# scipopt/SCIP-SDP

Measured on AMD Instinct MI355X. Metric: node-SDP solves/sec, dense block n x n with m vars (IPM iters/sec in iters_per_sec), higher is better.
Workload: dtype f64

## Files before the change

### include/hipsdp_units.h

```cpp
#ifndef HIPSDP_UNITS_H
#define HIPSDP_UNITS_H

#include "hipsdp.h"

#ifdef __cplusplus
extern "C" {
#endif

HIPSDP_API int  hipsdp_dgemm_selfcheck(int device, int M, int N, int K, int layB, int batch, int splitk, int flags, double beta,
   int* used_v2, long long* ndiff);
HIPSDP_API int  hipsdp_pass_at_unit(int device, int R, long long E, const double* A, const double* coef, double sa, const double* add, int split,
   double* out, int* chunks);
HIPSDP_API int  hipsdp_dgemm_selfcheck2(int device, int M, int N, int K, int layB, int batch, int splitk, int flags, double alpha, double beta,
   int reps, int* used, long long* ndiff, double* ms_tile, double* ms_fast);
HIPSDP_API int  hipsdp_gram_plan_info(int device, int M, long long K, int nslab, int* no, int* nd, int* nitems, double* span);
HIPSDP_API int  hipsdp_gram_selfcheck(int device, int M, long long K, int reps, int* used, double* maxdiff, long long* nrepro, double* ms_tile,
   double* ms_gram);
HIPSDP_API int  hipsdp_dgemm_selfcheck3(int device, int M, int N, int K, int layB, int batch, int splitk, int flags, double alpha, double beta,
   int reps, int* used, long long* ndiff, double* maxdiff, long long* nrepro, double* ms_tile, double* ms_fast);
HIPSDP_API int  hipsdp_tri_product_unit(int device, int mode, int M, int N, int K, int layB, int batch, int flags, const double* A,
   const double* B, double* Cio, int crows, int ldc, int* used);
HIPSDP_API int  hipsdp_tri_instance_force(int mode);
HIPSDP_API int  hipsdp_schur_identity_unit(int device, int m1, int n, const double* A, double ws_gbytes, int full_storage, double* Mx,
   double* flops);
HIPSDP_API int  hipsdp_schur_dense(int device, int m1, int n, const double* A, const double* X, const double* Zinv, double* Mx,
   double ws_gbytes);
HIPSDP_API int  hipsdp_schur_w(int device, int m1, int n, const double* A, const double* X, const double* Z, double* Mx);
HIPSDP_API int  hipsdp_schur_form_unit(int device, int form, int parts, int m1, int n, const double* A, const double* P, const double* Q,
   double ws_gbytes, double* Mx, int* used);
HIPSDP_API int  hipsdp_schur_small_unit(int device, int m1, int nblk, const int* ns, const double* const* A, const double* const* X,
   const double* const* Zinv, int q, const double* Dext, const double* x, const double* z, double* Mx, double* Lm, double* diagM, int* taken);
HIPSDP_API int  hipsdp_schur_shard_time(int device, int m1, int n, int nranks, int rank, int by_columns, int reps, double ws_gbytes, double* ms);
HIPSDP_API int  hipsdp_schur_var_share_time(int device, int m1, int n, int nranks, int rank, int cw, int reps, double* ms, double* a2a_bytes);
HIPSDP_API int  hipsdp_schur_sparse_unit(int device, int n, int m, long long nnz, const int* var, const int* row, const int* col,
   const double* val, const double* X, const double* Zinv, double* Mx);
HIPSDP_API int  hipsdp_schur_sparse_unit2(int device, int n, int m, long long nnz, const int* var, const int* row, const int* col,
   const double* val, const double* X, const double* Zinv, double* Mx, int kernel, int* took);
HIPSDP_API int  hipsdp_sparse_ops_unit(int device, int n, int m, long long nnz, const int* var, const int* row, const int* col,
   const double* val, const double* V, const double* coef, const double* base, double* outA, double* outAT);
HIPSDP_API int  hipsdp_mfma_peak(int device, double ms, double* tflops, double* ghz);
HIPSDP_API int  hipsdp_potrf(int device, int n, double* A, int* fail);
HIPSDP_API int  hipsdp_potrf_ex(int device, int n, double* A, int psd, int v1, double* dinv, int* regmask, int* fail);
HIPSDP_API int  hipsdp_potrs(int device, int n, const double* A, int nrhs, double* rhs);
HIPSDP_API int  hipsdp_potrs_seq(int device, int n, const double* A, int psd, int ncalls, const int* nrhs, const int* mode, double* rhs,
   int* regmask, int* fail);
HIPSDP_API int  hipsdp_potrf_small_unit(int device, int n, int pair, const double* base, const double* dir, double alpha, int set_flag,
   int want_gram, double* L, double* dinv, double* Mout, double* Linv, double* Gram, int* flag);
HIPSDP_API long long hipsdp_potrf_dinv_len(int n);
HIPSDP_API int  hipsdp_potrf_pair_unit(int device, int n, int pair, double* A, double* dinv, int* fail);
HIPSDP_API int  hipsdp_trial_pair_unit(int device, int n, int fused, int first, double alpha, double* io);
HIPSDP_API int  hipsdp_tail_after_solve2_unit(int device, int m, int fused, const double* rhs2, const double* u1, double* u2, double* wt,
   double* e2, double* e1);
HIPSDP_API int  hipsdp_tail_unpack3_unit(int device, int n, int fused, const double* pk, double* out);
HIPSDP_API int  hipsdp_tail_dz_unit(int device, int n, int fused, const double* pk, const double* P2, const double* Rd, double dtau, double eta,
   double* dZ);
HIPSDP_API int  hipsdp_tail_dirmat_unit(int device, int n, int fused, double s1, const double* Zinv, const double* X, const double* GZ, double* H,
   double* pk);
HIPSDP_API int  hipsdp_tail_sc_len(void);
HIPSDP_API int  hipsdp_tail_dir_unit(int device, int m, int n, int fused, const double* B, const double* H, const double* rhs2, const double* rp,
   const double* b, const double* u1, const double* u2, const double* par, double* sc, double* dy, double* dyt);
HIPSDP_API int  hipsdp_tail_dots_unit(int device, int m, int n, int fused, const double* a, const double* v, double* out);
HIPSDP_API int  hipsdp_trtri(int device, int n, const double* A, double* Linv);
HIPSDP_API int  hipsdp_lambda_min(int device, int n, const double* W, int steps, double* theta, double* resid);
HIPSDP_API int  hipsdp_lambda_min_scaled(int device, int n, const double* L, const double* D, int steps, double* theta, double* resid);
HIPSDP_API int  hipsdp_solve1_fits(int m, int q, int nblk, const int* ns);
HIPSDP_API int  hipsdp_solve1_class(int m, int nblk, const int* ns);
HIPSDP_API unsigned long long hipsdp_gram_gen_next(unsigned long long* counter);
HIPSDP_API int  hipsdp_gram_key_match_unit(int m_a, int nblk_a, const int* n_a, const int* form_a, const unsigned long long* gen_a,
   const long long* ws_a, int m_b, int nblk_b, const int* n_b, const int* form_b, const unsigned long long* gen_b, const long long* ws_b);
HIPSDP_API int  hipsdp_syev_many_unit(int device, int count, const int* ns, const double* A, double* lam, double* V, int* launches);
HIPSDP_API int  hipsdp_sparsecuts_unit(int device, int count, const int* ns, const double* Z, const double* v0, const double* maxeig,
   const int* sizes, const hipsdp_sparsecut_opts* opts, int* ncuts, double* eigvals, double* vecs, int* iters, int* flags);
HIPSDP_API int  hipsdp_sparsecuts_large_unit(int device, int n, const double* Z, const double* v0, double maxeig, int size,
   const hipsdp_sparsecut_opts* opts, int* ncuts, double* eigvals, double* vecs, int* iters, int* flags);
HIPSDP_API int  hipsdp_syevx_many_below_unit(int device, int count, const int* n, const double* A, double bound, int maxk, int cap, int* cnt,
   double* lam, double* V);
HIPSDP_API int  hipsdp_tridiag_unit(int device, int n, const double* A, double* d, double* e, double* Vrefl, double* tau);
HIPSDP_API int  hipsdp_tvec_unit(int device, int n, const double* d, const double* e, double* lam, double* Z);
HIPSDP_API int  hipsdp_syevr_many_unit(int device, int count, const int* n, const double* A, int cap, double* lam, double* V);
HIPSDP_API int  hipsdp_sparse_dump_unit(hipsdp_solver* solver, int block, long long* counts, int* voff, int* vrow, int* vcol, double* vval,
   int* poff, int* prow, int* pcol, int* pvar, double* pval, int* foff, int* frow, int* fcol, double* fval, int* soff, int* srow, int* sent);
HIPSDP_API int  hipsdp_onevar_unit(int device, int n, int count, const double* Z, const double* A, const double* shift, const int* kind,
   const double* lb, const double* ub, double feastol, int maxevals, int* status, double* optval, double* lmin, double* grad, int* evals);
HIPSDP_API int  hipsdp_onevar_all_unit(int device, int count, const int* n, const double* Z, const double* A, const double* shift,
   const int* kind, const double* lb, const double* ub, double feastol, int maxevals, int mid_cap,
   int* status, double* optval, double* lmin, double* grad, int* evals);
HIPSDP_API int  hipsdp_onevar_large_unit(int device, int count, const int* n, const double* Z, const double* A, const double* shift,
   const int* kind, const double* lb, const double* ub, double feastol, int maxevals, int wg_cap, int chunk,
   int* status, double* optval, double* lmin, double* grad, int* evals, int* rounds);
HIPSDP_API int  hipsdp_objs_fanout_unit(int device, int count, int m, int q, int nblk, const int* ns, const double* B, const double* b_own,
   int have_start, const double* y, const double* x, const double* z, const double* XZ, int gap, double guard, long long* lane_len,
   long long* offs, double* lanes, int* launches);
HIPSDP_API int  hipsdp_small_dir_block_unit(int device, int n, double c, double s1, const double* X, const double* R, const double* E,
   const double* Zinv, int recorded, double* out, int* pending);
HIPSDP_API int  hipsdp_small_lp_rows_unit(int device, int q, int m1, const double* Dext, const double* v, int mode, double eta, double sigmu,
   const double* x, const double* z, const double* rd, const double* elp, int recorded, double* out1, double* out2, int* pending);
HIPSDP_API int  hipsdp_small_apply_A_unit(int device, int m1, int nblk, const int* n2, const double* A, const double* V, int q,
   const double* Dext, const double* vlp, int epi, double scal, const double* vin, int recorded, double* out, double* vout, int* pending);
HIPSDP_API int  hipsdp_small_elementwise_unit(int device, int n, const int* nn, const double* par, int use_elp, const double* in,
   const double* xs, int recorded, double* o_lp, double* o_mul, double* o_ext, double* ys, int* pending);
HIPSDP_API int  hipsdp_small_gemv_t_unit(int device, int R, long long E, long long lda, const double* A, const double* coef, double sa,
   int add_mode, const double* add, int recorded, double* out, int* pending);
HIPSDP_API int  hipsdp_reductions_unit(int device, int kind, int count, const int* len, const int* slot, const int* accumulate,
   const double* a, const double* b, const double* c, int nslots, const double* preset, int recorded, double* out, int* pending);
HIPSDP_API int  hipsdp_small_solve_unit(int device, int m, const double* M, int form, int nrhs, long long ld, double* rhs, double* u2,
   double* wt, int* pending, int* fail);
HIPSDP_API int  hipsdp_gemv_t3_unit(int device, int R, long long E, long long lda, const double* A, const double* c, int fused, double* out,
   int* took);
HIPSDP_API int  hipsdp_pass_a_unit(int device, int R, long long E, long long lda, const double* A, int nv, const double* V, int voff,
   long long wsdoubles, double* out, int* info);

#ifdef __cplusplus
}
#endif

#endif
```

### scip-sdp_amd/binding.py

```python
import ctypes as C
import os
import numpy as np

_HERE = os.path.dirname(os.path.abspath(__file__))
LIBPATH = os.environ.get("HIPSDP_LIB", os.path.join(_HERE, "lib", "libhipsdp.so"))

STATUS_NAMES = {0: "optimal", 1: "dual_infeasible", 2: "dual_unbounded", 3: "both_infeasible", 4: "iterlimit",
                5: "numeric", 6: "timelimit", 7: "objlimit", -1: "unsolved"}


class Params(C.Structure):
    _fields_ = [("gaptol", C.c_double), ("feastol", C.c_double), ("infeastol", C.c_double), ("objlimit", C.c_double),
                ("timelimit", C.c_double), ("gamma", C.c_double), ("ws_gbytes", C.c_double), ("maxiter", C.c_int),
                ("verbose", C.c_int), ("lanczos_steps", C.c_int), ("settings", C.c_int), ("pabstol", C.c_double), ("preoptgap", C.c_double)]


class Info(C.Structure):
    _fields_ = [("status", C.c_int), ("iterations", C.c_int), ("pobj", C.c_double), ("dobj", C.c_double),
                ("pinf", C.c_double), ("dinf", C.c_double), ("dabs", C.c_double), ("gap", C.c_double), ("mu", C.c_double),
                ("tau", C.c_double), ("kappa", C.c_double), ("solve_seconds", C.c_double), ("schur_seconds", C.c_double),
                ("schur_flops", C.c_double), ("schur_calls", C.c_int), ("chol_fail", C.c_int), ("warm_started", C.c_int),
                ("settings_used", C.c_int), ("schur_flops_executed", C.c_double)]


# ... 700 lines not shown

def sparsecuts_unit(ns, Zs, v0s, maxeig, sizes, feastol, maxcuts, convtol=0, maxit=0, device=0):
    ns = [int(n) for n in ns]
    cnt = len(ns)
    cns = np.asarray(ns, dtype=np.int32)
    Z = _f64(np.concatenate([np.asarray(z, dtype=np.float64).reshape(-1) for z in Zs]))
    v0 = _f64(np.concatenate([np.asarray(v, dtype=np.float64).reshape(-1) for v in v0s]))
    me = _f64(maxeig)
    sizes = np.ascontiguousarray(sizes, dtype=np.int32)
    opts = SparsecutOpts(0.0, feastol, convtol, maxcuts, maxit)
    k, it, fl = (np.zeros(cnt, dtype=np.int32) for _ in range(3))
    ev = np.zeros(cnt * maxcuts)
    ve = np.zeros(maxcuts * sum(ns))
    rc = ulib().hipsdp_sparsecuts_unit(device, cnt, _ip(cns), _dp(Z), _dp(v0), _dp(me), _ip(sizes), C.byref(opts), _ip(k), _dp(ev), _dp(ve),
                                       _ip(it), _ip(fl))
    if rc != 0:
        raise RuntimeError("hipsdp_sparsecuts_unit: %d (%s)" % (rc, ulib().hipsdp_last_error()))
    out, off = [], 0
    for j, n in enumerate(ns):
        kj = int(k[j])
        out.append((kj, ev[j * maxcuts:j * maxcuts + kj].copy(), ve[off:off + kj * n].reshape(kj, n).copy(), int(it[j]), int(fl[j])))
        off += maxcuts * n
    return out


def eigencuts_all_stats():
    calls, launches, readbacks = C.c_longlong(0), C.c_longlong(0), C.c_longlong(0)
    _chk(lib().hipsdp_eigencuts_all_stats(C.byref(calls), C.byref(launches), C.byref(readbacks)), "hipsdp_eigencuts_all_stats")
    return calls.value, launches.value, readbacks.value


def eigencuts_all_large_stats():
    calls, launches, readbacks = C.c_longlong(0), C.c_longlong(0), C.c_longlong(0)
    _chk(lib().hipsdp_eigencuts_all_large_stats(C.byref(calls), C.byref(launches), C.byref(readbacks)), "hipsdp_eigencuts_all_large_stats")
    return calls.value, launches.value, readbacks.value


def syevx_many_below_unit(mats, bound, maxk, cap, device=0):
    mats = [np.asarray(a, dtype=np.float64) for a in mats]
    ns = np.ascontiguousarray([a.shape[0] for a in mats], dtype=np.int32)
    assert all(a.shape == (n, n) for a, n in zip(mats, ns))
    cat = _f64(np.concatenate([a.reshape(-1) for a in mats]))
    cnt = np.full(len(mats), -1, dtype=np.int32)
    mk = max(1, int(maxk))
    lam = np.zeros(len(mats) * mk)
    V = np.zeros(mk * int(sum(ns)))
    rc = ulib().hipsdp_syevx_many_below_unit(device, len(mats), _ip(ns), _dp(cat), C.c_double(bound), int(maxk), int(cap), _ip(cnt), _dp(lam),
                                             _dp(V))
    if rc != 0:
        raise RuntimeError("hipsdp_syevx_many_below_unit: %d (%s)" % (rc, ulib().hipsdp_last_error()))
    out, off = [], 0
    for j, n in enumerate(ns):
        kj = int(cnt[j])
        out.append((kj, lam[j * maxk:j * maxk + kj].copy(), V[off:off + kj * n].reshape(kj, n).copy()))
        off += maxk * int(n)
    return out



def _params(kw):
    p = Params()
    lib().hipsdp_default_params(C.byref(p))
    for k, v in (kw or {}).items():
        setattr(p, k, v)
    return p


def solve_many(solvers, params=None):
    n = len(solvers)
    if isinstance(params, (list, tuple)):
        if len(params) != n:
            raise ValueError("solve_many: %d params for %d solvers" % (len(params), n))
        plist = [_params(kw) for kw in params]
    else:
        plist = [_params(params)] * n
    hs = (C.c_void_p * max(n, 1))(*[s.h for s in solvers])
    ps = (Params * max(n, 1))(*plist)
    infos = (Info * max(n, 1))()
    rcs = (C.c_int * max(n, 1))()
    rc = lib().hipsdp_solve_many(n, hs, ps, infos, rcs)
    if rc != 0:
        raise RuntimeError("hipsdp_solve_many failed: rc=%d, per solver %s (%s)" %
                           (rc, list(rcs)[:n], lib().hipsdp_last_error().decode()))
    return [infos[i] for i in range(n)]


def solve_many_stats():
    launches = C.c_longlong(0)
    problems = C.c_longlong(0)
    _chk(lib().hipsdp_solve_many_stats(C.byref(launches), C.byref(problems)), "hipsdp_solve_many_stats")
    return launches.value, problems.value


def solve_objectives_stats():
    v = [C.c_longlong(0) for _ in range(3)]
    _chk(lib().hipsdp_solve_objectives_stats(*[C.byref(x) for x in v]), "hipsdp_solve_objectives_stats")
    return tuple(x.value for x in v)


def objs_fanout_unit(B, b_own, ns, q=0, start=None, gap=2, guard=-7.25):
    B = _f64(B)
    count, m = B.shape
    b_own = _f64(b_own)
    nsa = (C.c_int * max(len(ns), 1))(*[int(n) for n in ns])
    offs = np.zeros(4 + 2 * len(ns), dtype=np.int64)
    po = offs.ctypes.data_as(C.POINTER(C.c_longlong))
    ln = C.c_longlong(0)
    launches = C.c_int(0)
    if start is not None:
        y, x, z, X, Z = start
        y, x, z = _f64(y), _f64(x if q else np.zeros(1)), _f64(z if q else np.zeros(1))
        XZ = _f64(np.concatenate([np.concatenate([_f64(X[k]).ravel(), _f64(Z[k]).ravel()]) for k in range(len(ns))]))
        ptrs = (_dp(y), _dp(x), _dp(z), _dp(XZ))
    else:
        ptrs = (None, None, None, None)
    hs = 1 if start is not None else 0
    rc = ulib().hipsdp_objs_fanout_unit(0, count, m, q, len(ns), nsa, _dp(B), _dp(b_own), hs, *ptrs, gap, C.c_double(guard), C.byref(ln),
                                        po, None, None)
    if rc != 0:
        raise RuntimeError("hipsdp_objs_fanout_unit failed: rc=%d" % rc)
    lanes = np.zeros((count + 1, ln.value))
    rc = ulib().hipsdp_objs_fanout_unit(0, count, m, q, len(ns), nsa, _dp(B), _dp(b_own), hs, *ptrs, gap, C.c_double(guard), C.byref(ln),
                                        po, _dp(lanes), C.byref(launches))
    if rc != 0:
        raise RuntimeError("hipsdp_objs_fanout_unit failed: rc=%d (%s)" % (rc, ulib().hipsdp_last_error().decode()))
    return lanes, offs.copy(), launches.value


def solve1_fits(m, q, ns):
    a = (C.c_int * max(len(ns), 1))(*[int(n) for n in ns])
    return bool(ulib().hipsdp_solve1_fits(int(m), int(q), len(ns), a))


def solve1_class(m, ns):
    a = (C.c_int * max(len(ns), 1))(*[int(n) for n in ns])
    return ulib().hipsdp_solve1_class(int(m), len(ns), a)


def dgemm(A, B, layA=0, layB=1, alpha=1.0, beta=0.0, Cin=None, lower_only=False, splitk=0, device=0):
    A = _f64(A)
    B = _f64(B)
    M, K = (A.shape if layA == 0 else A.shape[::-1])
    N = B.shape[0] if layB == 0 else B.shape[1]
    Cout = np.zeros((M, N)) if Cin is None else _f64(Cin).copy()
    _chk(lib().hipsdp_dgemm(device, layA, layB, M, N, K, C.c_double(alpha), _dp(A), C.c_longlong(A.shape[1]), _dp(B),
                            C.c_longlong(B.shape[1]), C.c_double(beta), _dp(Cout), C.c_longlong(N), int(lower_only), splitk),
         "hipsdp_dgemm")
    return Cout


def schur_dense(A, X, Zinv, ws_gbytes=0.0, device=0):
    A = _f64(A)
    m1, n = A.shape[0], A.shape[1]
    X = _f64(X)
    Zinv = _f64(Zinv)
    Mx = np.zeros((m1, m1))
    _chk(ulib().hipsdp_schur_dense(device, m1, n, _dp(A), _dp(X), _dp(Zinv), _dp(Mx), C.c_double(ws_gbytes)),
         "hipsdp_schur_dense")
    return Mx


def schur_sparse_unit(n, m, coo, X, Zinv, device=0):
    var, row, col, val = coo
    var = np.ascontiguousarray(var, dtype=np.int32); row = np.ascontiguousarray(row, dtype=np.int32)
    col = np.ascontiguousarray(col, dtype=np.int32); val = _f64(val)
    X = _f64(X); Zinv = _f64(Zinv)
    Mx = np.zeros((m + 1, m + 1))
    _chk(ulib().hipsdp_schur_sparse_unit(device, n, m, C.c_longlong(len(val)), _ip(var), _ip(row), _ip(col), _dp(val), _dp(X), _dp(Zinv), _dp(Mx)),
         "hipsdp_schur_sparse_unit")
    return Mx


def _coo_i32(coo):
    var, row, col, val = coo
    return (np.ascontiguousarray(var, dtype=np.int32), np.ascontiguousarray(row, dtype=np.int32),
            np.ascontiguousarray(col, dtype=np.int32), _f64(val))


def schur_sparse_unit2(n, m, coo, X, Zinv, kernel=-1, device=0):
    var, row, col, val = _coo_i32(coo)
    X = _f64(X); Zinv = _f64(Zinv)
    Mx = np.zeros((m + 1, m + 1))
    took = C.c_int(-7)
    _chk(ulib().hipsdp_schur_sparse_unit2(device, n, m, C.c_longlong(len(val)), _ip(var), _ip(row), _ip(col), _dp(val), _dp(X), _dp(Zinv),
                                          _dp(Mx), int(kernel), C.byref(took)), "hipsdp_schur_sparse_unit2")
    return Mx, took.value


def sparse_ops_unit(n, m, coo, V=None, coef=None, base=None, device=0):
    var, row, col, val = _coo_i32(coo)
    outA = outAT = None
    pV = pc = pb = pA = pAT = None
    if V is not None:
        V = _f64(V)
        assert V.shape == (n, n)
        outA = np.full(m, np.nan)
        pV, pA = _dp(V), _dp(outA)
    if coef is not None:
        coef = _f64(coef)
        assert coef.shape == (m + 1,)
        base = np.zeros((n, n)) if base is None else _f64(base)
        assert base.shape == (n, n)
        outAT = np.full((n, n), np.nan)
        pc, pb, pAT = _dp(coef), _dp(base), _dp(outAT)
    _chk(ulib().hipsdp_sparse_ops_unit(device, n, m, C.c_longlong(len(val)), _ip(var), _ip(row), _ip(col), _dp(val), pV, pc, pb, pA, pAT),
         "hipsdp_sparse_ops_unit")
    return outA, outAT


def schur_w(A, X, Z, device=0):
    A = _f64(A)
    m1, n = A.shape[0], A.shape[1]
    X = _f64(X)
    Z = _f64(Z)
    Mx = np.zeros((m1, m1))
    _chk(ulib().hipsdp_schur_w(device, m1, n, _dp(A), _dp(X), _dp(Z), _dp(Mx)), "hipsdp_schur_w")
    return Mx


def schur_form_unit(form, A, P, Q, parts=1, ws_gbytes=0.0, device=0):
    A = _f64(A)
    m1, n = A.shape[0], A.shape[1]
    P = _f64(P); Q = _f64(Q)
    assert A.shape == (m1, n, n) and P.shape == (n, n) and Q.shape == (n, n)
    Mx = np.zeros((m1, m1))
    used = (C.c_int * 3)(0, 0, 0)
    _chk(ulib().hipsdp_schur_form_unit(device, form, parts, m1, n, _dp(A), _dp(P), _dp(Q), C.c_double(ws_gbytes), _dp(Mx), used),
         "hipsdp_schur_form_unit")
    return Mx, tuple(used)


def schur_small_unit(As, Xs, Zinvs, Dext=None, x=None, z=None, fill=0.0, device=0):
    As = [_f64(a) for a in As]; Xs = [_f64(a) for a in Xs]; Zinvs = [_f64(a) for a in Zinvs]
    nblk, m1 = len(As), As[0].shape[0]
    ns = np.array([a.shape[1] for a in As], dtype=np.int32)
    for k in range(nblk):
        assert As[k].shape == (m1, ns[k], ns[k]) and Xs[k].shape == (ns[k], ns[k]) and Zinvs[k].shape == (ns[k], ns[k])
    q = 0 if Dext is None else int(np.shape(Dext)[0])
    if q > 0:
        Dext = _f64(Dext); x = _f64(x); z = _f64(z)
        assert Dext.shape == (q, m1) and x.shape == (q,) and z.shape == (q,)
    arr = C.POINTER(C.c_double) * nblk
    pA, pX, pZ = arr(*[_dp(a) for a in As]), arr(*[_dp(a) for a in Xs]), arr(*[_dp(a) for a in Zinvs])
    m = m1 - 1
    Mx = np.full((m1, m1), fill)
    Lm = np.full(max(m * m, 1), fill)
    dg = np.full(max(m, 1), fill)
    taken = C.c_int(-1)
    _chk(ulib().hipsdp_schur_small_unit(device, m1, nblk, _ip(ns), pA, pX, pZ, q, _dp(Dext) if q else None, _dp(x) if q else None,
                                        _dp(z) if q else None, _dp(Mx), _dp(Lm), _dp(dg), C.byref(taken)), "hipsdp_schur_small_unit")
    return taken.value, Mx, Lm[:m * m].reshape(m, m), dg[:m]


def gram_plan_info(M, K, nslab=64, device=0):
    no, nd, ni = C.c_int(0), C.c_int(0), C.c_int(0)
    sp = C.c_double(0.0)
    rc = ulib().hipsdp_gram_plan_info(device, M, C.c_longlong(K), nslab, C.byref(no), C.byref(nd), C.byref(ni), C.byref(sp))
    return (no.value, nd.value, ni.value, sp.value) if rc == 0 else None


def dgemm_selfcheck(M, N, K, layB=1, batch=1, splitk=1, flags=0, beta=0.0, device=0):
    used = C.c_int(0)
    nd = C.c_longlong(0)
    _chk(ulib().hipsdp_dgemm_selfcheck(device, M, N, K, layB, batch, splitk, flags, C.c_double(beta), C.byref(used), C.byref(nd)),
         "hipsdp_dgemm_selfcheck")
    return used.value, nd.value


def dgemm_selfcheck2(M, N, K, layB=1, batch=1, splitk=1, flags=0, alpha=1.0, beta=0.0, reps=0, device=0):
    used = C.c_int(0)
    nd = C.c_longlong(0)
    t0, t1 = C.c_double(0.0), C.c_double(0.0)
    _chk(ulib().hipsdp_dgemm_selfcheck2(device, M, N, K, layB, batch, splitk, flags, C.c_double(alpha), C.c_double(beta), reps,
                                       C.byref(used), C.byref(nd), C.byref(t0), C.byref(t1)), "hipsdp_dgemm_selfcheck2")
    return used.value, nd.value, t0.value, t1.value


def dgemm_selfcheck3(M, N, K, layB=1, batch=1, splitk=1, flags=0, alpha=1.0, beta=0.0, reps=0, device=0):
    used = C.c_int(0)
    nd, nr = C.c_longlong(0), C.c_longlong(0)
    md, t0, t1 = C.c_double(0.0), C.c_double(0.0), C.c_double(0.0)
    _chk(ulib().hipsdp_dgemm_selfcheck3(device, M, N, K, layB, batch, splitk, flags, C.c_double(alpha), C.c_double(beta), reps,
                                       C.byref(used), C.byref(nd), C.byref(md), C.byref(nr), C.byref(t0), C.byref(t1)), "hipsdp_dgemm_selfcheck3")
    return used.value, nd.value, md.value, nr.value, t0.value, t1.value


def tri_product_unit(A, B, flags, mode, layB=1, sentinel=None, pad_rows=0, pad_cols=0, device=0):
    A = _f64(A); B = _f64(B)
    M, K = A.shape
    batch = B.shape[0]
    N = B.shape[2] if layB == 1 else B.shape[1]
    assert B.shape == ((batch, K, N) if layB == 1 else (batch, N, K))
    Cio = np.full((batch, M + pad_rows, N + pad_cols), np.nan if sentinel is None else sentinel)
    used = (C.c_int * 2)(0, 0)
    _chk(ulib().hipsdp_tri_product_unit(device, mode, M, N, K, layB, batch, flags, _dp(A), _dp(B), _dp(Cio), M + pad_rows, N + pad_cols, used),
         "hipsdp_tri_product_unit")
    return Cio, tuple(used)


def tri_instance_force(mode):
    return ulib().hipsdp_tri_instance_force(mode)


def gram_selfcheck(M, K, reps=0, device=0):
    used = C.c_int(0)
    nr = C.c_longlong(0)
    md, t0, t1 = C.c_double(0.0), C.c_double(0.0), C.c_double(0.0)
    _chk(ulib().hipsdp_gram_selfcheck(device, M, C.c_longlong(K), reps, C.byref(used), C.byref(md), C.byref(nr), C.byref(t0), C.byref(t1)),
         "hipsdp_gram_selfcheck")
    return used.value, md.value, nr.value, t0.value, t1.value


def schur_identity_unit(A, Mx=None, ws_gbytes=0.0, full_storage=False, device=0):
    A = _f64(A)
    m1, n = A.shape[0], A.shape[1]
    Mx = np.zeros((m1, m1)) if Mx is None else _f64(Mx).copy()
    fl = C.c_double(0.0)
    _chk(ulib().hipsdp_schur_identity_unit(device, m1, n, _dp(A), C.c_double(ws_gbytes), int(full_storage), _dp(Mx), C.byref(fl)),
         "hipsdp_schur_identity_unit")
    return Mx, fl.value


def potrf(A, device=0):
    L = _f64(A).copy()
    fail = C.c_int(0)
    _chk(ulib().hipsdp_potrf(device, L.shape[0], _dp(L), C.byref(fail)), "hipsdp_potrf")
    return np.tril(L), fail.value


def potrf_ex(A, psd=False, v1=False, device=0):
    L = _f64(A).copy()
    n = L.shape[0]
    dinv = np.zeros(((n + 63) // 64) * 4096)
    mask = np.zeros(n, dtype=np.int32)
    fail = C.c_int(0)
    _chk(ulib().hipsdp_potrf_ex(device, n, _dp(L), int(psd), int(v1), _dp(dinv), _ip(mask), C.byref(fail)), "hipsdp_potrf_ex")
    return L, dinv, mask, fail.value


def potrs(A, rhs, device=0):
    A = _f64(A)
    r = _f64(rhs).copy()
    r2 = r.reshape(-1, A.shape[0])
    _chk(ulib().hipsdp_potrs(device, A.shape[0], _dp(A), r2.shape[0], _dp(r2)), "hipsdp_potrs")
    return r2.reshape(r.shape)


def potrs_seq(A, calls, psd=False, device=0):
    A = _f64(A)
    n = A.shape[0]
    nc = len(calls)
    slab = np.zeros((max(nc, 1), 4, n))
    nrhs = np.zeros(max(nc, 1), dtype=np.int32)
    mode = np.zeros(max(nc, 1), dtype=np.int32)
    for c, (md, r) in enumerate(calls):
        r = _f64(r).reshape(-1, n)
        nrhs[c], mode[c] = r.shape[0], md
        slab[c, :min(r.shape[0], 4)] = r[:4]
    mask = np.zeros(n, dtype=np.int32)
    fail = C.c_int(0)
    _chk(ulib().hipsdp_potrs_seq(device, n, _dp(A), int(psd), nc, _ip(nrhs), _ip(mode), _dp(slab), _ip(mask), C.byref(fail)),
         "hipsdp_potrs_seq")
    return [slab[c, :nrhs[c]].copy() for c in range(nc)], mask, fail.value


def potrf_small_unit(base, dir=None, alpha=0.0, pair=False, set_flag=False, want_gram=False, device=0):
    base = _f64(base)
    n = base.shape[-1]
    npb = 2 if pair else 1
    assert base.size == npb * n * n
    d = None if dir is None else _f64(dir)
    assert d is None or d.size == base.size
    shp = (2, n, n) if pair else (n, n)
    out = {"L": np.zeros(shp), "dinv": np.zeros((2, 64, 64) if pair else (64, 64)), "Mout": np.zeros(shp), "Linv": np.zeros(shp),
           "Gram": np.zeros(shp) if want_gram else None}
    flag = np.zeros(2, dtype=np.int32)
    _chk(ulib().hipsdp_potrf_small_unit(device, n, int(pair), _dp(base), None if d is None else _dp(d), C.c_double(alpha), int(set_flag),
                                        int(want_gram), _dp(out["L"]), _dp(out["dinv"]), _dp(out["Mout"]), _dp(out["Linv"]),
                                        None if not want_gram else _dp(out["Gram"]), _ip(flag)), "hipsdp_potrf_small_unit")
    out["flag"] = flag.copy() if pair else int(flag[0])
    return out


def potrf_pair_unit(A2, pair=True, device=0):
    L = _f64(A2).copy()
    n = L.shape[-1]
    assert L.shape == (2, n, n)
    ulib().hipsdp_potrf_dinv_len.restype = C.c_longlong
    nd = int(ulib().hipsdp_potrf_dinv_len(n))
    dinv = np.zeros((2, nd))
    fail = np.zeros(2, dtype=np.int32)
    _chk(ulib().hipsdp_potrf_pair_unit(device, n, int(pair), _dp(L), _dp(dinv), _ip(fail)), "hipsdp_potrf_pair_unit")
    return L, dinv, fail


def trial_pair_unit(arrays, alpha, fused=True, first=True, device=0):
    io = _f64(arrays).copy()
    n = io.shape[-1]
    assert io.shape == (8, n, n)
    _chk(ulib().hipsdp_trial_pair_unit(device, n, int(fused), int(first), C.c_double(alpha), _dp(io)), "hipsdp_trial_pair_unit")
    return io


def _packed_len(n):
    t = n * (n + 1) // 2
    return t + (t & 1)


def tail_after_solve2_unit(rhs2, u1, fused, device=0):
    rhs2, u1 = _f64(rhs2), _f64(u1)
    m = u1.size
    assert rhs2.size == 2 * m
    u2, wt, e2, e1 = np.zeros(m), np.zeros(m + 1), np.zeros(m + 1), np.zeros(m + 1)
    _chk(ulib().hipsdp_tail_after_solve2_unit(device, m, int(fused), _dp(rhs2), _dp(u1), _dp(u2), _dp(wt), _dp(e2), _dp(e1)),
         "hipsdp_tail_after_solve2_unit")
    return u2, wt, e2, e1


def tail_unpack3_unit(pk, n, fused, device=0):
    pk = _f64(pk)
    assert pk.shape == (3, _packed_len(n))
    out = np.zeros((3, n, n))
    _chk(ulib().hipsdp_tail_unpack3_unit(device, n, int(fused), _dp(pk), _dp(out)), "hipsdp_tail_unpack3_unit")
    return out


def tail_dz_unit(pk, P2, Rd, dtau, eta, fused, device=0):
    pk, P2, Rd = _f64(pk), _f64(P2), _f64(Rd)
    n = P2.shape[0]
    assert pk.size == _packed_len(n) and P2.shape == Rd.shape == (n, n)
    dZ = np.zeros((n, n))
    _chk(ulib().hipsdp_tail_dz_unit(device, n, int(fused), _dp(pk), _dp(P2), _dp(Rd), C.c_double(dtau), C.c_double(eta), _dp(dZ)),
         "hipsdp_tail_dz_unit")
    return dZ


def tail_dirmat_unit(s1, Zinv, X, GZ, fused, device=0):
    Zinv, X, GZ = _f64(Zinv), _f64(X), _f64(GZ)
    n = X.shape[0]
    H, pk = np.zeros((n, n)), np.zeros(_packed_len(n))
    _chk(ulib().hipsdp_tail_dirmat_unit(device, n, int(fused), C.c_double(s1), _dp(Zinv), _dp(X), _dp(GZ), _dp(H), _dp(pk)),
         "hipsdp_tail_dirmat_unit")
    return H, pk


def tail_dir_unit(B, H, rhs2, rp, b, u1, u2, par, sc, fused, device=0):
    B, H = _f64(B), _f64(H)
    vs = [_f64(v) for v in (rhs2, rp, b, u1, u2)]
    m, n = vs[0].size, B.shape[0]
    par = _f64(par)
    sc = _f64(sc).copy()
    assert par.size == 6 and sc.size == ulib().hipsdp_tail_sc_len() and all(v.size == m for v in vs) and B.shape == H.shape == (n, n)
    dy, dyt = np.zeros(m), np.zeros(m + 1)
    _chk(ulib().hipsdp_tail_dir_unit(device, m, n, int(fused), _dp(B), _dp(H), _dp(vs[0]), _dp(vs[1]), _dp(vs[2]), _dp(vs[3]), _dp(vs[4]),
                                     _dp(par), _dp(sc), _dp(dy), _dp(dyt)), "hipsdp_tail_dir_unit")
    return sc, dy, dyt


def tail_sc_len():
    return int(ulib().hipsdp_tail_sc_len())


def tail_dots_unit(a, v, fused, device=0):
    a, v = _f64(a), _f64(v)
    n = int(round(np.sqrt(a.shape[1])))
    assert a.shape == (3, n * n) and v.shape[0] == 2
    out = np.zeros(3)
    _chk(ulib().hipsdp_tail_dots_unit(device, v.shape[1], n, int(fused), _dp(a), _dp(v), _dp(out)), "hipsdp_tail_dots_unit")
    return out


def _opt(a):
    return None if a is None else _dp(a)


def small_dir_block_unit(c, s1, X, R, E, Zinv, recorded, device=0):
    X, R, Zinv = _f64(X), _f64(R), _f64(Zinv)
    E = None if E is None else _f64(E)
    n = X.shape[0]
    assert X.shape == R.shape == Zinv.shape == (n, n) and (E is None or E.shape == (n, n))
    out, pend = np.zeros((n, n)), C.c_int(-1)
    _chk(ulib().hipsdp_small_dir_block_unit(device, n, C.c_double(c), C.c_double(s1), _dp(X), _dp(R), _opt(E), _dp(Zinv), int(recorded),
                                            _dp(out), C.byref(pend)), "hipsdp_small_dir_block_unit")
    return out, pend.value


def small_lp_rows_unit(Dext, v, mode, eta, sigmu, x, z, rd, elp, recorded, device=0):
    Dext, v, x, z, rd = _f64(Dext), _f64(v), _f64(x), _f64(z), _f64(rd)
    elp = None if elp is None else _f64(elp)
    q, m1 = Dext.shape
    assert v.size == m1 and x.size == z.size == rd.size == q and (elp is None or elp.size == q)
    o1, o2, pend = np.zeros(q), np.zeros(q), C.c_int(-1)
    _chk(ulib().hipsdp_small_lp_rows_unit(device, q, m1, _dp(Dext), _dp(v), int(mode), C.c_double(eta), C.c_double(sigmu), _dp(x), _dp(z),
                                          _dp(rd), _opt(elp), int(recorded), _dp(o1), _dp(o2), C.byref(pend)), "hipsdp_small_lp_rows_unit")
    return o1, o2, pend.value


def small_apply_A_unit(As, Vs, Dext, vlp, epi, scal, vin, recorded, device=0):
    As = [_f64(a) for a in As]
    Vs = [_f64(v).ravel() for v in Vs]
    m1 = As[0].shape[0]
    n2 = np.array([a.shape[1] for a in As], dtype=np.int32)
    assert all(a.shape[0] == m1 for a in As) and all(v.size == k for v, k in zip(Vs, n2))
    A = np.concatenate([a.ravel() for a in As])
    V = np.concatenate(Vs)
    Dext, vlp, vin = _f64(Dext).reshape(-1, m1), _f64(vlp), _f64(vin)
    q = Dext.shape[0]
    assert vlp.size == q and vin.size == m1 - 1
    out, vout, pend = np.zeros(m1), np.zeros(m1 - 1), C.c_int(-1)
    _chk(ulib().hipsdp_small_apply_A_unit(device, m1, len(As), _ip(n2), _dp(A), _dp(V), q, _dp(Dext), _dp(vlp), int(epi), C.c_double(scal),
                                          _dp(vin), int(recorded), _dp(out), _dp(vout), C.byref(pend)), "hipsdp_small_apply_A_unit")
    return out, vout, pend.value


def small_elementwise_unit(vecs, par, xs, ys, nn, use_elp, recorded, device=0):
    vecs, par, xs, ys = _f64(vecs), _f64(par), _f64(xs), _f64(ys).copy()
    nn = np.ascontiguousarray(nn, dtype=np.int32)
    n = vecs.shape[1]
    assert vecs.shape == (6, n) and par.size == 5 and nn.size == 3 and xs.size == ys.size == int(nn.sum())
    o_lp, o_mul, o_ext, pend = np.zeros(n), np.zeros(n), np.zeros(n + 1), C.c_int(-1)
    _chk(ulib().hipsdp_small_elementwise_unit(device, n, _ip(nn), _dp(par), int(use_elp), _dp(vecs), _dp(xs), int(recorded), _dp(o_lp),
                                              _dp(o_mul), _dp(o_ext), _dp(ys), C.byref(pend)), "hipsdp_small_elementwise_unit")
    return o_lp, o_mul, o_ext, ys, pend.value


def small_gemv_t_unit(A, E, coef, sa, add, add_mode, recorded, device=0):
    A, coef = _f64(A), _f64(coef)
    R, lda = A.shape
    add = None if add is None else _f64(add)
    assert coef.size == R and 1 <= E <= lda and (add_mode == 0 or add.size == E)
    out, pend = np.zeros(E), C.c_int(-1)
    _chk(ulib().hipsdp_small_gemv_t_unit(device, R, C.c_longlong(E), C.c_longlong(lda), _dp(A), _dp(coef), C.c_double(sa), int(add_mode),
                                         _opt(add), int(recorded), _dp(out), C.byref(pend)), "hipsdp_small_gemv_t_unit")
    return out, pend.value


def reductions_unit(kind, lens, slots, accumulate, a, b, c, preset, recorded, device=0):
    lens, slots, accumulate = (np.ascontiguousarray(v, dtype=np.int32) for v in (lens, slots, accumulate))
    a, b, c, preset = _f64(a), _f64(b), _f64(c), _f64(preset)
    assert lens.size == slots.size == accumulate.size and a.size == b.size == c.size == int(lens.sum())
    out, pend = np.zeros(preset.size), C.c_int(-1)
    _chk(ulib().hipsdp_reductions_unit(device, int(kind), lens.size, _ip(lens), _ip(slots), _ip(accumulate), _dp(a), _dp(b), _dp(c),
                                       preset.size, _dp(preset), int(recorded), _dp(out), C.byref(pend)), "hipsdp_reductions_unit")
    return out, pend.value


def small_solve_unit(M, rhs, form, ld=None, device=0):
    M = _f64(M)
    m = M.shape[0]
    rhs = _f64(rhs).copy()
    pend, fail = C.c_int(-1), C.c_int(-1)
    if form == 0:
        nrhs, ld = rhs.shape
        _chk(ulib().hipsdp_small_solve_unit(device, m, _dp(M), 0, nrhs, C.c_longlong(ld), _dp(rhs), None, None, C.byref(pend),
                                            C.byref(fail)), "hipsdp_small_solve_unit")
        return rhs, pend.value, fail.value
    assert rhs.size == 2 * m
    u2, wt = np.zeros(m), np.zeros(m + 1)
    _chk(ulib().hipsdp_small_solve_unit(device, m, _dp(M), 1, 0, C.c_longlong(0), _dp(rhs), _dp(u2), _dp(wt), C.byref(pend),
                                        C.byref(fail)), "hipsdp_small_solve_unit")
    return rhs, u2, wt, fail.value


def gemv_t3_unit(A, E, c, fused, device=0):
    A, c = _f64(A), _f64(c)
    R, lda = A.shape
    assert c.shape == (3, R) and 1 <= E <= lda
    out, took = np.zeros((3, E)), C.c_int(-1)
    _chk(ulib().hipsdp_gemv_t3_unit(device, R, C.c_longlong(E), C.c_longlong(lda), _dp(A), _dp(c), int(fused), _dp(out), C.byref(took)),
         "hipsdp_gemv_t3_unit")
    return out, took.value


def pass_a_unit(A, E, V, voff=0, wsdoubles=0, device=0):
    A, V = _f64(A), _f64(V)
    R, lda = A.shape
    nv = V.shape[0]
    assert V.shape == (nv, E) and 1 <= E <= lda
    out = np.zeros((nv, R))
    info = np.zeros(2, dtype=np.int32)
    _chk(ulib().hipsdp_pass_a_unit(device, R, C.c_longlong(E), C.c_longlong(lda), _dp(A), nv, _dp(V), int(voff), C.c_longlong(wsdoubles),
                                   _dp(out), _ip(info)), "hipsdp_pass_a_unit")
    return out, int(info[0]), bool(info[1])


def trtri(A, device=0):
    A = _f64(A)
    Li = np.zeros_like(A)
    _chk(ulib().hipsdp_trtri(device, A.shape[0], _dp(A), _dp(Li)), "hipsdp_trtri")
    return Li


def lambda_min(W, steps=0, device=0):
    W = _f64(W)
    th = C.c_double(0.0)
    rs = C.c_double(0.0)
    _chk(ulib().hipsdp_lambda_min(device, W.shape[0], _dp(W), steps, C.byref(th), C.byref(rs)), "hipsdp_lambda_min")
    return th.value, rs.value


def syev(A, device=0):
    A = _f64(A)
    n = A.shape[0]
    lam = np.zeros(n)
    V = np.zeros((n, n))
    _chk(lib().hipsdp_syev(device, n, _dp(A), _dp(lam), _dp(V)), "hipsdp_syev")
# ... 164 lines not shown
```

### scip-sdp_amd/csrc/gram.hip

```cpp
#include "hs_common.h"
#include <stdlib.h>
#include <stdio.h>
#include <map>
#include <mutex>
#include <utility>
#include <tuple>
#include <vector>
#include <queue>
#include <algorithm>
#include <functional>

typedef double gr_v4d __attribute__((ext_vector_type(4)));
typedef __attribute__((address_space(3))) void* gr_lds_ptr;
typedef const __attribute__((address_space(1))) void* gr_gbl_ptr;

#define GR_BT   128
#define GR_BKS  8
#define GR_NS   4
#define GR_OPSZ (GR_BT * GR_BKS)
#define GR_SLOT (2 * GR_OPSZ)
#define GR_GPS  4
#define GR_UNI(x) __builtin_amdgcn_readfirstlane(x)

__device__ __attribute__((aligned(16))) double hs_gr_zero[2] = {0.0, 0.0};

struct gram_item
{
   int ti, tj;
   int k0, k1;
   int slab;
   int pad;
};

struct gram_args
{
   const double* W;
   long long ldw;
   int M;
   double* ws;
   const gram_item* items;
   const int* off;
};

template<int N> __device__ __forceinline__ void gr_wait_vm()
{
   asm volatile("s_waitcnt vmcnt(%0)" :: "n"(N) : "memory");
}

__device__ __forceinline__ double gr_frag(const double* __restrict__ img, int t, int ks, int lane)
{
   const int k = 4 * ks + (lane >> 4);
   return img[t * 128 + (k >> 1) * 32 + (lane & 15) * 2 + (k & 1)];
}

__global__ void __launch_bounds__(256, 2) hs_gram_kernel(gram_args g)
{
   extern __shared__ __attribute__((aligned(1024))) double gr_smem[];
   const int tid = threadIdx.x, lane = tid & 63;
   const int wave = GR_UNI(tid >> 6);
   const int wm = wave >> 1, wn = wave & 1;
   const int wg = (blockIdx.x & 7) * 64 + (blockIdx.x >> 3);
   const int lbeg = GR_UNI(g.off[wg]), lend = GR_UNI(g.off[wg + 1]);
   const int ar = lane & 15, ac = lane >> 4;

   gr_v4d acc[16];
#pragma unroll
   for (int i = 0; i < 16; ++i)
      acc[i] = (gr_v4d){0.0, 0.0, 0.0, 0.0};

   int dcol[9];
   bool dlo[9];
#pragma unroll
   for (int k = 0; k < 9; ++k)
   {
      dlo[k] = k <= wave;
      dcol[k] = k <= wave ? k : k - wave - 1;
   }

   const double* pa[2]; const double* pb[2];
   int ck0 = 0, ck1 = 0;
   pa[0] = pa[1] = pb[0] = pb[1] = hs_gr_zero;
   auto piece = [&](int st, int k) __attribute__((always_inline))
   {
      const int i = k & 1;
      const int pc = wave * 2 + i;
      const int K0 = ck0 + GR_BKS * st;
      const double* src = (K0 + 2 * ac < ck1) ? (k < 2 ? pa[i] : pb[i]) + K0 : hs_gr_zero;
      __builtin_amdgcn_global_load_lds((gr_gbl_ptr) src, (gr_lds_ptr) (gr_smem + (st & 3) * GR_SLOT + (k < 2 ? 0 : GR_OPSZ) + pc * 128), 16, 0, 0);
   };

   auto run_off = [&](int nst) __attribute__((always_inline))
   {
      double f0a[4], f0b[4], f1a[4], f1b[4];
      auto landed_frags = [&](double (&fa)[4], double (&fb)[4]) __attribute__((always_inline))
      {
#pragma unroll
         for (int i = 0; i < 4; ++i)
            asm volatile("" : "+v"(fa[i]), "+v"(fb[i]));
      };
#pragma unroll
      for (int st = 0; st < GR_NS; ++st)
#pragma unroll
         for (int k = 0; k < 4; ++k)
            piece(st, k);
      gr_wait_vm<3 * 4>();
      __builtin_amdgcn_s_barrier();
#pragma unroll
      for (int i = 0; i < 4; ++i)
      {
         f0a[i] = gr_frag(gr_smem, 4 * wm + i, 0, lane);
         f0b[i] = gr_frag(gr_smem + GR_OPSZ, 4 * wn + i, 0, lane);
      }
      asm volatile("s_waitcnt lgkmcnt(0)" ::: "memory");
      landed_frags(f0a, f0b);
      for (int s = 0; s < nst; ++s)
      {
         const double* sa = gr_smem + (s & 3) * GR_SLOT;
         const double* sn = gr_smem + ((s + 1) & 3) * GR_SLOT;
         __builtin_amdgcn_sched_barrier(0);
#pragma unroll
         for (int i = 0; i < 4; ++i)
         {
            f1a[i] = gr_frag(sa, 4 * wm + i, 1, lane);
            f1b[i] = gr_frag(sa + GR_OPSZ, 4 * wn + i, 1, lane);
         }
#pragma unroll
         for (int i = 0; i < 4; ++i)
#pragma unroll
            for (int j = 0; j < 4; ++j)
               acc[4 * i + j] = __builtin_amdgcn_mfma_f64_16x16x4f64(f0a[i], f0b[j], acc[4 * i + j], 0, 0, 0);
#pragma unroll
         for (int q = 0; q < 8; ++q)
         {
            __builtin_amdgcn_sched_group_barrier(0x008, 1, 0);
            __builtin_amdgcn_sched_group_barrier(0x100, 1, 0);
         }
         __builtin_amdgcn_sched_group_barrier(0x008, 8, 0);
         __builtin_amdgcn_sched_barrier(0);
         asm volatile("s_waitcnt lgkmcnt(0)" ::: "memory");
         landed_frags(f1a, f1b);
         gr_wait_vm<2 * 4>();
         __builtin_amdgcn_s_barrier();
         __builtin_amdgcn_sched_barrier(0);
         acc[0] = __builtin_amdgcn_mfma_f64_16x16x4f64(f1a[0], f1b[0], acc[0], 0, 0, 0);
         acc[1] = __builtin_amdgcn_mfma_f64_16x16x4f64(f1a[0], f1b[1], acc[1], 0, 0, 0);
#pragma unroll
         for (int k = 0; k < 4; ++k)
         {
            __builtin_amdgcn_sched_barrier(0);
            piece(s + GR_NS, k);
            acc[2 + k] = __builtin_amdgcn_mfma_f64_16x16x4f64(f1a[(2 + k) >> 2], f1b[(2 + k) & 3], acc[2 + k], 0, 0, 0);
         }
         __builtin_amdgcn_sched_barrier(0);
#pragma unroll
         for (int i = 0; i < 4; ++i)
         {
            f0a[i] = gr_frag(sn, 4 * wm + i, 0, lane);
            f0b[i] = gr_frag(sn + GR_OPSZ, 4 * wn + i, 0, lane);
         }
#pragma unroll
         for (int k = 6; k < 16; ++k)
            acc[k] = __builtin_amdgcn_mfma_f64_16x16x4f64(f1a[k >> 2], f1b[k & 3], acc[k], 0, 0, 0);
#pragma unroll
         for (int q = 0; q < 8; ++q)
         {
            __builtin_amdgcn_sched_group_barrier(0x008, 1, 0);
            __builtin_amdgcn_sched_group_barrier(0x100, 1, 0);
         }
         __builtin_amdgcn_sched_barrier(0);
         asm volatile("s_waitcnt lgkmcnt(0)" ::: "memory");
         landed_frags(f0a, f0b);
      }
   };

   auto run_diag = [&](int nst) __attribute__((always_inline))
   {
      double a0[2], b0[9], a1[2], b1[9];
      auto read_set = [&](double (&a)[2], double (&b)[9], const double* img, int ks) __attribute__((always_inline))
      {
         a[0] = gr_frag(img, wave, ks, lane);
         a[1] = gr_frag(img, 7 - wave, ks, lane);
#pragma unroll
         for (int k = 0; k < 9; ++k)
            b[k] = gr_frag(img, dcol[k], ks, lane);
      };
      auto landed_set = [&](double (&a)[2], double (&b)[9]) __attribute__((always_inline))
      {
         asm volatile("" : "+v"(a[0]), "+v"(a[1]));
#pragma unroll
         for (int k = 0; k < 9; ++k)
            asm volatile("" : "+v"(b[k]));
      };
      auto mfma_k = [&](const double (&a)[2], const double (&b)[9], int k) __attribute__((always_inline))
      {
         const double av = dlo[k] ? a[0] : a[1];
         acc[k] = __builtin_amdgcn_mfma_f64_16x16x4f64(av, b[k], acc[k], 0, 0, 0);
      };
#pragma unroll
      for (int st = 0; st < GR_NS; ++st)
#pragma unroll
         for (int k = 0; k < 2; ++k)
            piece(st, k);
      gr_wait_vm<3 * 2>();
      __builtin_amdgcn_s_barrier();
      read_set(a0, b0, gr_smem, 0);
      asm volatile("s_waitcnt lgkmcnt(0)" ::: "memory");
      landed_set(a0, b0);
      for (int s = 0; s < nst; ++s)
      {
         const double* sa = gr_smem + (s & 3) * GR_SLOT;
         const double* sn = gr_smem + ((s + 1) & 3) * GR_SLOT;
         __builtin_amdgcn_sched_barrier(0);
         read_set(a1, b1, sa, 1);
#pragma unroll
         for (int k = 0; k < 9; ++k)
            mfma_k(a0, b0, k);
#pragma unroll
         for (int q = 0; q < 5; ++q)
         {
            __builtin_amdgcn_sched_group_barrier(0x008, 1, 0);
            __builtin_amdgcn_sched_group_barrier(0x100, 2, 0);
         }
         __builtin_amdgcn_sched_group_barrier(0x008, 1, 0);
         __builtin_amdgcn_sched_group_barrier(0x100, 1, 0);
         __builtin_amdgcn_sched_group_barrier(0x008, 3, 0);
         __builtin_amdgcn_sched_barrier(0);
         asm volatile("s_waitcnt lgkmcnt(0)" ::: "memory");
         landed_set(a1, b1);
         gr_wait_vm<2 * 2>();
         __builtin_amdgcn_s_barrier();
         __builtin_amdgcn_sched_barrier(0);
         mfma_k(a1, b1, 0);
         mfma_k(a1, b1, 1);
#pragma unroll
         for (int k = 0; k < 2; ++k)
         {
            __builtin_amdgcn_sched_barrier(0);
            piece(s + GR_NS, k);
            mfma_k(a1, b1, 2 + k);
         }
         __builtin_amdgcn_sched_barrier(0);
         read_set(a0, b0, sn, 0);
#pragma unroll
         for (int k = 4; k < 9; ++k)
            mfma_k(a1, b1, k);
#pragma unroll
         for (int q = 0; q < 4; ++q)
         {
            __builtin_amdgcn_sched_group_barrier(0x008, 1, 0);
            __builtin_amdgcn_sched_group_barrier(0x100, 3, 0);
         }
         __builtin_amdgcn_sched_group_barrier(0x008, 1, 0);
         __builtin_amdgcn_sched_barrier(0);
         asm volatile("s_waitcnt lgkmcnt(0)" ::: "memory");
         landed_set(a0, b0);
      }
   };

   for (int cur = lbeg; cur < lend; ++cur)
   {
      const gram_item it = g.items[cur];
      const int cti = GR_UNI(it.ti), ctj = GR_UNI(it.tj), cslab = GR_UNI(it.slab);
      ck0 = GR_UNI(it.k0); ck1 = GR_UNI(it.k1);
      const int nst = (ck1 - ck0 + GR_BKS - 1) / GR_BKS;
      const bool diag = cti == ctj;
#pragma unroll
      for (int i = 0; i < 2; ++i)
      {
         const int pc = wave * 2 + i;
         int row = cti * GR_BT + pc * 16 + ar;
         if ( row > g.M - 1 ) row = g.M - 1;
         pa[i] = g.W + (long long) row * g.ldw + 2 * ac;
         int rowb = ctj * GR_BT + pc * 16 + ar;
         if ( rowb > g.M - 1 ) rowb = g.M - 1;
         pb[i] = g.W + (long long) rowb * g.ldw + 2 * ac;
      }
      if ( diag )
         run_diag(nst);
      else
         run_off(nst);
      gr_wait_vm<0>();
      {
         double* C = g.ws + (long long) cslab * (long long) g.M * g.M;
         const int m0 = cti * GR_BT, n0 = ctj * GR_BT;
         if ( !diag )
         {
#pragma unroll
            for (int i = 0; i < 4; ++i)
#pragma unroll
               for (int r = 0; r < 4; ++r)
               {
                  const int row = m0 + wm * 64 + 16 * i + (lane >> 4) + 4 * r;
                  if ( row < g.M )
                  {
                     double* cr = C + (long long) row * g.M + n0 + wn * 64 + (lane & 15);
#pragma unroll
                     for (int j = 0; j < 4; ++j)
                        cr[16 * j] = acc[4 * i + j][r];
                  }
               }
         }
         else
         {
#pragma unroll
            for (int k = 0; k < 9; ++k)
            {
               const int rs = dlo[k] ? wave : 7 - wave;
#pragma unroll
               for (int r = 0; r < 4; ++r)
               {
                  const int row = m0 + 16 * rs + (lane >> 4) + 4 * r;
                  const int col = m0 + 16 * dcol[k] + (lane & 15);
                  if ( row < g.M && col < g.M )
                     C[(long long) row * g.M + col] = acc[k][r];
               }
            }
         }
#pragma unroll
         for (int i = 0; i < 16; ++i)
            acc[i] = (gr_v4d){0.0, 0.0, 0.0, 0.0};
      }
      __syncthreads();
   }
}

__global__ void hs_gram_reduce_kernel(int M, int no, int nd, const double* __restrict__ ws, double* __restrict__ C, long long ldc, double alpha, double beta)
{
   const long long MM = (long long) M * M;
   for (long long e = (long long) blockIdx.x * blockDim.x + threadIdx.x; e < MM; e += (long long) gridDim.x * blockDim.x)
   {
      const int r = (int) (e / M), c = (int) (e - (long long) r * M);
      if ( c > r )
         continue;
      const int ns = (r / GR_BT == c / GR_BT) ? nd : no;
      double s = 0.0;
      for (int k = 0; k < ns; ++k)
         s += ws[(long long) k * MM + e];
      double* q = C + (long long) r * ldc + c;
      *q = beta != 0.0 ? alpha * s + beta * (*q) : alpha * s;
   }
}

namespace {

struct GramPlan
{
   std::vector<gram_item> items;
   std::vector<int> off;
   int no, nd;
   double span;
   double executed;
   gram_item* dev;
   int* devoff;
};

#define GR_DIAG_COST 0.72

bool gr_make_plan(GramPlan& P, int tm, long long K, int so, int sd)
{
   const int noff = tm * (tm - 1) / 2;
   const double cd = GR_DIAG_COST;
   if ( so < 1 || sd < 1 )
      return false;
   long long lo = (K + so - 1) / so, ld = (K + sd - 1) / sd;
   lo = ((lo + GR_BKS - 1) / GR_BKS) * GR_BKS;
   ld = ((ld + GR_BKS - 1) / GR_BKS) * GR_BKS;
   if ( (long long) (so - 1) * lo + 8 * GR_BKS > K || (long long) (sd - 1) * ld + 8 * GR_BKS > K )
      return false;
   std::vector<gram_item> all;
   for (int s = 0; s < so; ++s)
      for (int i = 1; i < tm; ++i)
         for (int j = 0; j < i; ++j)
         {
            gram_item it = {i, j, (int) (s * lo), (int) ((s + 1) * lo < K ? (s + 1) * lo : K), s, 0};
            all.push_back(it);
         }
   for (int s = 0; s < sd; ++s)
      for (int i = 0; i < tm; ++i)
      {
         gram_item it = {i, i, (int) (s * ld), (int) ((s + 1) * ld < K ? (s + 1) * ld : K), s, 0};
         all.push_back(it);
      }
   (void) noff;
   std::stable_sort(all.begin(), all.end(), [](const gram_item& a, const gram_item& b) { return a.k0 < b.k0; });
   auto cost = [&](const gram_item& it) { return (it.ti == it.tj ? cd : 1.0) * (double) (it.k1 - it.k0) / (double) K; };
   double total = 0.0;
   P.executed = 0.0;
   for (const gram_item& it : all)
   {
      total += cost(it);
      P.executed += 2048.0 * (double) ((it.k1 - it.k0 + GR_BKS - 1) / GR_BKS) * (it.ti == it.tj ? 72.0 : 128.0);
   }
   P.items.clear();
   P.off.assign(513, 0);
   P.span = 0.0;
   size_t pos = 0;
   double done = 0.0;
   for (int x = 0; x < 8; ++x)
   {
      std::vector<gram_item> mine;
      const double upto = total * (double) (x + 1) / 8.0;
      while ( pos < all.size() && (x == 7 || done + 0.5 * cost(all[pos]) <= upto) )
      {
         done += cost(all[pos]);
         mine.push_back(all[pos++]);
      }
      std::vector<size_t> order(mine.size());
      for (size_t i = 0; i < order.size(); ++i) order[i] = i;
      std::stable_sort(order.begin(), order.end(), [&](size_t a, size_t b) { return cost(mine[a]) > cost(mine[b]); });
      std::vector<std::vector<gram_item> > lists(64);
      std::vector<double> load(64, 0.0);
      for (size_t i : order)
      {
         int w = 0;
         for (int v = 1; v < 64; ++v)
            if ( load[v] < load[w] ) w = v;
         load[w] += cost(mine[i]);
         lists[w].push_back(mine[i]);
      }
      for (int w = 0; w < 64; ++w)
      {
         std::stable_sort(lists[w].begin(), lists[w].end(), [](const gram_item& a, const gram_item& b) { return a.k0 < b.k0; });
         P.off[64 * x + w] = (int) P.items.size();
         for (const gram_item& it : lists[w])
            P.items.push_back(it);
         if ( load[w] > P.span ) P.span = load[w];
      }
   }
   P.off[512] = (int) P.items.size();
   P.no = so; P.nd = sd;
   return true;
}

GramPlan* gr_plan(int M, long long K, int nslab)
{
   static std::mutex mu;
   static std::map<std::tuple<int, int, long long, int>, GramPlan*> tab;
   int dev = 0;
   if ( hipGetDevice(&dev) != hipSuccess )
      return NULL;
   std::lock_guard<std::mutex> lk(mu);
   const auto key = std::make_tuple(dev, M, K, nslab);
   auto f = tab.find(key);
   if ( f != tab.end() )
      return f->second;
   const int tm = (M + GR_BT - 1) / GR_BT;
   const int ntile = tm * (tm + 1) / 2;
   GramPlan* best = NULL;
   GramPlan cand;
   cand.dev = NULL; cand.devoff = NULL;
   auto consider = [&](bool ok, double penalty)
   {
      if ( !ok )
         return;
      cand.span += penalty;
      if ( best == NULL || cand.span < best->span )
      {
         if ( best == NULL )
            best = new GramPlan();
         *best = cand;
      }
   };
   const int noff = ntile - tm;
   for (int so = 1; so <= nslab && (long long) noff * so + tm <= 512; ++so)
      for (int sd = (so + 1) / 2; sd <= so && (long long) noff * so + (long long) tm * sd <= 512; ++sd)
         consider(gr_make_plan(cand, tm, K, so, sd), 0.24 * ((double) so * noff + (double) sd * tm) / (double) K);
   if ( best != NULL )
   {
      const int sold = hs_dgemm_pick_xcd_slices(ntile, K);
      const double oldspan = (double) (((long long) ntile * sold + 511) / 512) / (double) sold;
      if ( best->span * 1.03 > oldspan || best->items.size() < 256 )
      {
         delete best;
         best = NULL;
      }
   }
   if ( best != NULL )
   {
      gram_item* d = NULL;
      int* doff = NULL;
      if ( hipMalloc((void**) &d, best->items.size() * sizeof(gram_item)) != hipSuccess
         || hipMemcpy(d, best->items.data(), best->items.size() * sizeof(gram_item), hipMemcpyHostToDevice) != hipSuccess
         || hipMalloc((void**) &doff, 513 * sizeof(int)) != hipSuccess
         || hipMemcpy(doff, best->off.data(), 513 * sizeof(int), hipMemcpyHostToDevice) != hipSuccess )
      {
         if ( d != NULL ) (void) hipFree(d);
         if ( doff != NULL ) (void) hipFree(doff);
         delete best;
         return NULL;
      }
      best->dev = d;
      best->devoff = doff;
   }
   tab[key] = best;
   return best;
}

}

static int gr_taken = 0;

int hs_gram_taken(void)
{
   return __atomic_load_n(&gr_taken, __ATOMIC_RELAXED);
}

int hs_gram_try(hipStream_t stream, int M, long long K, const double* W, long long ldw, double* C, long long ldc, double alpha, double beta,
   double* ws, int nslab, double* executed)
{
   if ( ws == NULL || nslab < 2 || M < 256 || K < 16384 )
      return 0;
   if ( (ldw & 1) || (K & 1) || (((uintptr_t) W) & 15) || K > 2000000000LL )
      return 0;
   if ( nslab > 64 ) nslab = 64;
   GramPlan* P = gr_plan(M, K, nslab);
   if ( P == NULL || P->dev == NULL || P->items.size() < 256 )
      return 0;
   gram_args g;
   g.W = W; g.ldw = ldw; g.M = M; g.ws = ws; g.items = P->dev; g.off = P->devoff;
   static hs_attr_mask attr_done;
   const size_t smem = (size_t) GR_NS * GR_SLOT * sizeof(double);
   if ( hs_func_max_lds(reinterpret_cast<const void*>(&hs_gram_kernel), (int) smem, &attr_done) != HS_OK )
      return -HS_ERR_HIP;
   hipLaunchKernelGGL(hs_gram_kernel, dim3(512), dim3(256), smem, stream, g);
   if ( hipGetLastError() != hipSuccess )
      return -HS_ERR_HIP;
   {
      int blocks = (int) (((long long) M * M + 255) / 256);
      if ( blocks > 2048 ) blocks = 2048;
      hipLaunchKernelGGL(hs_gram_reduce_kernel, dim3(blocks), dim3(256), 0, stream, M, P->no, P->nd, ws, C, ldc, alpha, beta);
      if ( hipGetLastError() != hipSuccess )
         return -HS_ERR_HIP;
   }
   if ( executed != NULL )
      *executed = P->executed;
   (void) __atomic_add_fetch(&gr_taken, 1, __ATOMIC_RELAXED);
   return 1;
}

int hs_gram_plan_info(int M, long long K, int nslab, int* no, int* nd, int* nitems, double* span)
{
   GramPlan* P = gr_plan(M, K, nslab > 64 ? 64 : nslab);
   if ( P == NULL )
      return 0;
   *no = P->no; *nd = P->nd; *nitems = (int) P->items.size(); *span = P->span;
   return 1;
}
```

### scip-sdp_amd/csrc/hs_common.h

```cpp
#ifndef HS_COMMON_H
#define HS_COMMON_H

#include <hip/hip_runtime.h>
#include <stddef.h>
#include <stdint.h>

#define HS_OK            0
#define HS_ERR_NODEVICE  1
#define HS_ERR_HIP       2
#define HS_ERR_ARG       3
#define HS_ERR_NOMEM     4
#define HS_ERR_NUMERIC   5

#define HS_HIP(call)                                                                       \
   do {                                                                                    \
      hipError_t hs_e_ = (call);                                                           \
      if ( hs_e_ != hipSuccess ) {                                                         \
         hs_record_hip_error(hs_e_, #call, __FILE__, __LINE__);                            \
         return (hs_e_ == hipErrorOutOfMemory) ? HS_ERR_NOMEM : HS_ERR_HIP;                \
      }                                                                                    \
   } while (0)

#define HS_CALL(call)                                                                      \
   do {                                                                                    \
      int hs_r_ = (call);                                                                  \
      if ( hs_r_ != HS_OK )                                                                \
         return hs_r_;                                                                     \
   } while (0)

#define HS_LAUNCH_CHECK()                                                                  \
   do {                                                                                    \
      hipError_t e_ = hipGetLastError();                                                   \
      if ( e_ != hipSuccess ) {                                                            \
         hs_record_hip_error(e_, "kernel launch", __FILE__, __LINE__);                     \
         return HS_ERR_HIP;                                                                \
      }                                                                                    \
   } while (0)

void hs_record_hip_error(hipError_t e, const char* what, const char* file, int line);
const char* hs_last_error(void);

struct hs_attr_mask { unsigned long long bits[2]; };
int hs_func_max_lds(const void* fn, int bytes, hs_attr_mask* done);
int hs_func_attr_sets(int device);
int hs_device_cus(void);

int hs_pool_alloc(void** p, size_t bytes);
void hs_pool_free(void* p);
void hs_pool_trim(void);

#define HS_KC 0
#define HS_MC 1

#define HS_GEMM_LOWER     1
#define HS_GEMM_A_LOWTRI  2
#define HS_GEMM_B_LOWTRI  4
#define HS_GEMM_A_UPTRI 256
#define HS_GEMM_XCD       8
#define HS_GEMM_TILE64  128
#define HS_GEMM_NOFAST   64
#define HS_GEMM_UPPER    32
#define HS_GEMM_REMAP    16
int hs_dgemm_pick_xcd_slices(long long ntile, long long K);

struct hs_gemm_args
{
   int            M, N, K;
   int            layA, layB;
   const double*  A;
   long long      lda;
   long long      strideA;
   const double*  B;
   long long      ldb;
   long long      strideB;
   double*        C;
   long long      ldc;
   long long      strideC;
   double         alpha, beta;
   int            batch;
   int            flags;
   int            splitk;
   double*        ws;
};

int hs_dgemm(hipStream_t stream, const hs_gemm_args* args);
int hs_dgemm2_try(hipStream_t stream, const hs_gemm_args* args, int kchunk);
int hs_dgemm2_enable(int on);
int hs_dgemm2_paired_taken(void);
int hs_dgemm2_wide_force(int mode);
int hs_dgemm2_tri5_forced(void);
int hs_gram_taken(void);

int hs_gram_try(hipStream_t stream, int M, long long K, const double* W, long long ldw, double* C, long long ldc, double alpha, double beta,
   double* ws, int nslab, double* executed);
int hs_gram_plan_info(int M, long long K, int nslab, int* no, int* nd, int* nitems, double* span);

int hs_dgemm3_try(hipStream_t stream, const hs_gemm_args* args);

double hs_mfma_flops_total(void);
void   hs_mfma_flops_add(double flops);
int hs_dgemm2_tri5_eligible(const hs_gemm_args* a);
int hs_dgemm2_tri5_wide(const hs_gemm_args* a);
double hs_gemm_executed_flops(const hs_gemm_args* a, int BT, int kstage, int kchunk, int persistent);

int hs_dgemm_pick_splitk(int M, int N, int K, int lowerOnly);

#endif
```

### scip-sdp_amd/csrc/units.hip

```cpp
#include "hs_kernels.h"
#include "hs_chunks.h"
#include "hs_gram_cache.h"
#include "../../include/hipsdp.h"
#include "../../include/hipsdp_units.h"
#include <vector>
#include <algorithm>
#include <cstring>
#include <cstdlib>

namespace {

struct DevBuf
{
   double* p;
   DevBuf() : p(NULL) {}
   ~DevBuf() { if ( p ) (void) hipFree(p); }
   int alloc(long long n) { if ( n <= 0 ) n = 1; hipError_t e = hipMalloc((void**) &p, (size_t) n * sizeof(double)); if ( e != hipSuccess ) { hs_record_hip_error(e, "hipMalloc", __FILE__, __LINE__); return e == hipErrorOutOfMemory ? HS_ERR_NOMEM : HS_ERR_HIP; } return HS_OK; }
   int up(const double* h, long long n) { if ( n <= 0 ) return HS_OK; hipError_t e = hipMemcpy(p, h, (size_t) n * sizeof(double), hipMemcpyHostToDevice); if ( e != hipSuccess ) { hs_record_hip_error(e, "H2D", __FILE__, __LINE__); return HS_ERR_HIP; } return HS_OK; }
   int down(double* h, long long n) { if ( n <= 0 ) return HS_OK; hipError_t e = hipMemcpy(h, p, (size_t) n * sizeof(double), hipMemcpyDeviceToHost); if ( e != hipSuccess ) { hs_record_hip_error(e, "D2H", __FILE__, __LINE__); return HS_ERR_HIP; } return HS_OK; }
};

int pick_device(int device)
{
   int nd = 0;
// ... 41 lines not shown
   if ( m > 0.0 )
      atomicMax(out, (unsigned long long) __double_as_longlong(m));
}

__global__ void k_unit_tri(int rows, int cols, long long stride, int batch, double* __restrict__ x)
{
   const long long per = (long long) rows * cols;
   for (long long e = (long long) blockIdx.x * blockDim.x + threadIdx.x; e < per * batch; e += (long long) gridDim.x * blockDim.x)
   {
      const long long b = e / per, w = e - b * per;
      const int r = (int) (w / cols), c = (int) (w - (long long) r * cols);
      if ( c > r )
         x[b * stride + w] = 0.0;
   }
}

__global__ void k_unit_tri_upper(int rows, int cols, double* __restrict__ x)
{
   const long long per = (long long) rows * cols;
   for (long long e = (long long) blockIdx.x * blockDim.x + threadIdx.x; e < per; e += (long long) gridDim.x * blockDim.x)
   {
      const int r = (int) (e / cols), c = (int) (e - (long long) r * cols);
      if ( c < r )
         x[e] = 0.0;
   }
}

static int dgemm_selfcheck_impl(int device, int M, int N, int K, int layB, int batch, int splitk, int flags, double alpha, double beta,
   int reps, int* used, long long* ndiff, double* ms_tile, double* ms_fast, double* maxdiff = NULL, long long* nrepro = NULL)
{
   HS_CALL( pick_device(device) );
   if ( M <= 0 || N <= 0 || K <= 0 || batch < 1 )
      return HIPSDP_ERR_ARG;
   const long long na = (long long) M * K, nb = (long long) N * K, nc = (long long) M * N;
   const long long sB = (batch > 1) ? nb : 0;
   DevBuf dA, dB, dC1, dC2, dW;
   unsigned long long* dn = NULL;
   HS_CALL( dA.alloc(na) ); HS_CALL( dB.alloc(batch > 1 ? nb * batch : nb) ); HS_CALL( dC1.alloc(nc * batch) ); HS_CALL( dC2.alloc(nc * batch) );
   if ( splitk > 1 )
      HS_CALL( dW.alloc((long long) splitk * nc) );
   HS_HIP( hipMalloc((void**) &dn, sizeof(unsigned long long)) );
   HS_HIP( hipMemset(dn, 0, sizeof(unsigned long long)) );
   hipLaunchKernelGGL(k_unit_fill, dim3(1024), dim3(256), 0, 0, na, 11ULL, dA.p);
   hipLaunchKernelGGL(k_unit_fill, dim3(1024), dim3(256), 0, 0, batch > 1 ? nb * batch : nb, 23ULL, dB.p);
   hipLaunchKernelGGL(k_unit_fill, dim3(1024), dim3(256), 0, 0, nc * batch, 37ULL, dC1.p);
   if ( flags & HS_GEMM_A_LOWTRI )
      hipLaunchKernelGGL(k_unit_tri, dim3(1024), dim3(256), 0, 0, M, K, 0LL, 1, dA.p);
   if ( (flags & HS_GEMM_B_LOWTRI) && layB == HS_MC )
      hipLaunchKernelGGL(k_unit_tri, dim3(1024), dim3(256), 0, 0, K, N, nb, batch, dB.p);
   if ( flags & HS_GEMM_A_UPTRI )
      hipLaunchKernelGGL(k_unit_tri_upper, dim3(1024), dim3(256), 0, 0, M, K, dA.p);
   HS_HIP( hipMemcpy(dC2.p, dC1.p, (size_t) (nc * batch) * sizeof(double), hipMemcpyDeviceToDevice) );
   hs_gemm_args g = {M, N, K, HS_KC, layB, dA.p, K, 0, dB.p, layB == HS_KC ? (long long) K : (long long) N, sB, dC1.p, N, nc, alpha, beta,
      batch, flags, splitk, dW.p};
   hipEvent_t e0 = NULL, e1 = NULL;
   if ( reps > 0 && (hipEventCreate(&e0) != hipSuccess || hipEventCreate(&e1) != hipSuccess) )
      return HS_ERR_HIP;
   auto timed = [&](double* ms) -> int
   {
      if ( reps <= 0 || ms == NULL || beta != 0.0 )
         return HS_OK;
      int rc = HS_OK;
      for (int w = 0; w < 2 && rc == HS_OK; ++w)
         rc = hs_dgemm(0, &g);
      (void) hipEventRecord(e0, 0);
      for (int r = 0; r < reps && rc == HS_OK; ++r)
         rc = hs_dgemm(0, &g);
      (void) hipEventRecord(e1, 0);
      if ( rc == HS_OK && hipEventSynchronize(e1) != hipSuccess )
         rc = HS_ERR_HIP;
      float t = 0.f;
      if ( rc == HS_OK && hipEventElapsedTime(&t, e0, e1) != hipSuccess )
         rc = HS_ERR_HIP;
      *ms = (double) t / reps;
      return rc;
   };
   int rc = HS_OK;
   hs_dgemm2_enable(0);
   rc = hs_dgemm(0, &g);
   if ( rc == HS_OK )
      rc = timed(ms_tile);
   const int before = hs_dgemm2_enable(1);
   g.C = dC2.p;
   if ( splitk > 1 )
      hipLaunchKernelGGL(k_unit_fill, dim3(1024), dim3(256), 0, 0, (long long) splitk * nc, 51ULL, dW.p);
   if ( rc == HS_OK )
      rc = hs_dgemm(0, &g);
   const int after = hs_dgemm2_enable(1);
   if ( rc == HS_OK )
      rc = timed(ms_fast);
   if ( rc == HS_OK && hipDeviceSynchronize() != hipSuccess )
      rc = HS_ERR_HIP;
   unsigned long long hn = 0;
   if ( rc == HS_OK )
   {
      hipLaunchKernelGGL(k_unit_maxdiff, dim3(1024), dim3(256), 0, 0, nc * batch, dC1.p, dC2.p, dn);
      if ( hipMemcpy(&hn, dn, sizeof(hn), hipMemcpyDeviceToHost) != hipSuccess )
         rc = HS_ERR_HIP;
   }
   if ( rc == HS_OK && nrepro != NULL )
   {
      DevBuf dC3;
      unsigned long long hr = 0;
      rc = dC3.alloc(nc * batch);
      if ( rc == HS_OK && hipMemcpy(dC3.p, dC1.p, (size_t) (nc * batch) * sizeof(double), hipMemcpyDeviceToDevice) != hipSuccess )
         rc = HS_ERR_HIP;
      if ( rc == HS_OK && beta != 0.0 )
      {
         hipLaunchKernelGGL(k_unit_fill, dim3(1024), dim3(256), 0, 0, nc * batch, 37ULL, dC3.p);
         hipLaunchKernelGGL(k_unit_fill, dim3(1024), dim3(256), 0, 0, nc * batch, 37ULL, dC2.p);
         g.C = dC2.p;
         rc = hs_dgemm(0, &g);
      }
      g.C = dC3.p;
      if ( rc == HS_OK )
         rc = hs_dgemm(0, &g);
      if ( rc == HS_OK && hipMemset(dn, 0, sizeof(unsigned long long)) != hipSuccess )
         rc = HS_ERR_HIP;
      if ( rc == HS_OK )
      {
         hipLaunchKernelGGL(k_unit_maxdiff, dim3(1024), dim3(256), 0, 0, nc * batch, dC2.p, dC3.p, dn);
         if ( hipMemcpy(&hr, dn, sizeof(hr), hipMemcpyDeviceToHost) != hipSuccess )
            rc = HS_ERR_HIP;
      }
      *nrepro = (long long) hr;
      g.C = dC2.p;
   }
   if ( rc == HS_OK && maxdiff != NULL )
   {
      unsigned long long bits = 0;
      if ( hipMemset(dn, 0, sizeof(unsigned long long)) != hipSuccess )
         rc = HS_ERR_HIP;
      hipLaunchKernelGGL(k_unit_maxabsdiff, dim3(1024), dim3(256), 0, 0, nc * batch, dC1.p, dC2.p, dn);
      if ( rc == HS_OK && hipMemcpy(&bits, dn, sizeof(bits), hipMemcpyDeviceToHost) != hipSuccess )
         rc = HS_ERR_HIP;
      memcpy(maxdiff, &bits, sizeof(double));
   }
   (void) hipFree(dn);
   if ( e0 != NULL ) (void) hipEventDestroy(e0);
   if ( e1 != NULL ) (void) hipEventDestroy(e1);
   HS_CALL( rc );
   *used = after - before > 0 ? 1 : 0;
   *ndiff = (long long) hn;
   return HIPSDP_OK;
}

extern "C" int hipsdp_dgemm_selfcheck(int device, int M, int N, int K, int layB, int batch, int splitk, int flags, double beta,
   int* used_v2, long long* ndiff)
{
   int used = 0;
   HS_CALL( dgemm_selfcheck_impl(device, M, N, K, layB, batch, splitk, flags, 1.25, beta, 0, &used, ndiff, NULL, NULL) );
   *used_v2 = used & 1;
   return HIPSDP_OK;
}

extern "C" int hipsdp_dgemm_selfcheck2(int device, int M, int N, int K, int layB, int batch, int splitk, int flags, double alpha, double beta,
   int reps, int* used, long long* ndiff, double* ms_tile, double* ms_fast)
{
   return dgemm_selfcheck_impl(device, M, N, K, layB, batch, splitk, flags, alpha, beta, reps, used, ndiff, ms_tile, ms_fast);
}

extern "C" int hipsdp_dgemm_selfcheck3(int device, int M, int N, int K, int layB, int batch, int splitk, int flags, double alpha, double beta,
   int reps, int* used, long long* ndiff, double* maxdiff, long long* nrepro, double* ms_tile, double* ms_fast)
{
   return dgemm_selfcheck_impl(device, M, N, K, layB, batch, splitk, flags, alpha, beta, reps, used, ndiff, ms_tile, ms_fast, maxdiff, nrepro);
}

extern "C" int hipsdp_tri_product_unit(int device, int mode, int M, int N, int K, int layB, int batch, int flags, const double* A,
   const double* B, double* Cio, int crows, int ldc, int* used)
{
   HS_CALL( pick_device(device) );
   if ( mode < -1 || mode > 1 || M < 1 || N < 1 || K < 1 || batch < 1 || (layB != HS_MC && layB != HS_KC) || A == NULL || B == NULL || Cio == NULL
      || crows < M || ldc < N || used == NULL )
      return HIPSDP_ERR_ARG;
   const long long na = (long long) M * K, nb = (long long) N * K, nc = (long long) crows * ldc;
   DevBuf dA, dB, dC;
   HS_CALL( dA.alloc(na) ); HS_CALL( dB.alloc(nb * batch) ); HS_CALL( dC.alloc(nc * batch) );
   HS_CALL( dA.up(A, na) ); HS_CALL( dB.up(B, nb * batch) ); HS_CALL( dC.up(Cio, nc * batch) );
   hs_gemm_args g = {M, N, K, HS_KC, layB, dA.p, K, 0, dB.p, layB == HS_KC ? (long long) K : (long long) N, nb, dC.p, ldc, nc, 1.0, 0.0,
      batch, flags, 1, NULL};
   const int t5 = hs_dgemm2_paired_taken();
   const int tw = hs_dgemm2_wide_force(mode);
   int rc = hs_dgemm(0, &g);
   if ( rc == HS_OK && hipDeviceSynchronize() != hipSuccess ) rc = HS_ERR_HIP;
   used[1] = hs_dgemm2_wide_force(-1) - tw;
   used[0] = hs_dgemm2_paired_taken() - t5;
   HS_CALL( rc );
   HS_CALL( dC.down(Cio, nc * batch) );
   return HIPSDP_OK;
}

extern "C" int hipsdp_tri_instance_force(int mode)
{
   return hs_dgemm2_wide_force(mode);
}

__global__ void k_unit_lowdiff(int M, const double* __restrict__ a, const double* __restrict__ b, unsigned long long* __restrict__ out)
{
   double m = 0.0;
   unsigned long long cnt = 0;
   const long long MM = (long long) M * M;
   for (long long e = (long long) blockIdx.x * blockDim.x + threadIdx.x; e < MM; e += (long long) gridDim.x * blockDim.x)
   {
      const int r = (int) (e / M), c = (int) (e - (long long) r * M);
      if ( c > r )
         continue;
      const double d = fabs(a[e] - b[e]);
      if ( !(d <= m) )
         m = (d != d) ? 1e300 : d;
      if ( __double_as_longlong(a[e]) != __double_as_longlong(b[e]) )
         ++cnt;
   }
   if ( m > 0.0 )
      atomicMax(out, (unsigned long long) __double_as_longlong(m));
   if ( cnt )
      atomicAdd(out + 1, cnt);
}

extern "C" int hipsdp_gram_selfcheck(int device, int M, long long K, int reps, int* used, double* maxdiff, long long* nrepro, double* ms_tile,
   double* ms_gram)
{
   HS_CALL( pick_device(device) );
   if ( M <= 0 || K <= 0 || used == NULL || maxdiff == NULL || nrepro == NULL )
      return HIPSDP_ERR_ARG;
   const long long MM = (long long) M * M;
   const long long tm = (M + 127) / 128;
   int sk = hs_dgemm_pick_xcd_slices(tm * (tm + 1) / 2, K);
   const int nslab = 64;
   DevBuf dW, dC1, dC2, dC3, dS;
   unsigned long long* dn = NULL;
   HS_CALL( dW.alloc((long long) M * K) ); HS_CALL( dC1.alloc(MM) ); HS_CALL( dC2.alloc(MM) ); HS_CALL( dC3.alloc(MM) ); HS_CALL( dS.alloc((long long) nslab * MM) );
   HS_HIP( hipMalloc((void**) &dn, 2 * sizeof(unsigned long long)) );
   hipLaunchKernelGGL(k_unit_fill, dim3(1024), dim3(256), 0, 0, (long long) M * K, 11ULL, dW.p);
   hipLaunchKernelGGL(k_unit_fill, dim3(1024), dim3(256), 0, 0, MM, 37ULL, dC1.p);
   hipLaunchKernelGGL(k_unit_fill, dim3(1024), dim3(256), 0, 0, MM, 37ULL, dC2.p);
   hipLaunchKernelGGL(k_unit_fill, dim3(1024), dim3(256), 0, 0, MM, 37ULL, dC3.p);
   hipLaunchKernelGGL(k_unit_fill, dim3(1024), dim3(256), 0, 0, (long long) nslab * MM, 51ULL, dS.p);
   hs_gemm_args g3 = {M, M, (int) K, HS_KC, HS_KC, dW.p, K, 0, dW.p, K, 0, dC1.p, M, 0, 1.0, 1.0, 1, HS_GEMM_LOWER | HS_GEMM_XCD | HS_GEMM_NOFAST, sk, dS.p};
   int rc = hs_dgemm(0, &g3);
   int r2 = 0;
   double ex = 0.0;
   if ( rc == HS_OK )
   {
      hipLaunchKernelGGL(k_unit_fill, dim3(1024), dim3(256), 0, 0, (long long) nslab * MM, 52ULL, dS.p);
      r2 = hs_gram_try(0, M, K, dW.p, K, dC2.p, M, 1.0, 1.0, dS.p, nslab, &ex);
      if ( r2 < 0 ) rc = -r2;
   }
   if ( rc == HS_OK && r2 == 1 )
   {
      hipLaunchKernelGGL(k_unit_fill, dim3(1024), dim3(256), 0, 0, (long long) nslab * MM, 53ULL, dS.p);
      r2 = hs_gram_try(0, M, K, dW.p, K, dC3.p, M, 1.0, 1.0, dS.p, nslab, &ex);
      if ( r2 < 0 ) rc = -r2;
   }
   *used = r2 == 1 ? 1 : 0;
   *maxdiff = 0.0; *nrepro = 0;
   unsigned long long h[2] = {0, 0};
   if ( rc == HS_OK && r2 == 1 )
   {
      if ( hipMemset(dn, 0, 2 * sizeof(unsigned long long)) != hipSuccess ) rc = HS_ERR_HIP;
      hipLaunchKernelGGL(k_unit_lowdiff, dim3(1024), dim3(256), 0, 0, M, dC1.p, dC2.p, dn);
      if ( rc == HS_OK && hipMemcpy(h, dn, sizeof(h), hipMemcpyDeviceToHost) != hipSuccess ) rc = HS_ERR_HIP;
      memcpy(maxdiff, &h[0], sizeof(double));
      if ( rc == HS_OK && hipMemset(dn, 0, 2 * sizeof(unsigned long long)) != hipSuccess ) rc = HS_ERR_HIP;
      hipLaunchKernelGGL(k_unit_lowdiff, dim3(1024), dim3(256), 0, 0, M, dC2.p, dC3.p, dn);
      if ( rc == HS_OK && hipMemcpy(h, dn, sizeof(h), hipMemcpyDeviceToHost) != hipSuccess ) rc = HS_ERR_HIP;
      *nrepro = (long long) h[1];
   }
   if ( rc == HS_OK && reps > 0 && ms_tile != NULL && ms_gram != NULL )
   {
      hipEvent_t e0, e1;
      HS_HIP( hipEventCreate(&e0) ); HS_HIP( hipEventCreate(&e1) );
      for (int which = 0; which < 2 && rc == HS_OK; ++which)
      {
         for (int it = -2; it < reps && rc == HS_OK; ++it)
         {
            if ( it == 0 )
               (void) hipEventRecord(e0, 0);
            if ( which == 0 )
               rc = hs_dgemm(0, &g3);
            else if ( r2 == 1 )
            {
               const int r = hs_gram_try(0, M, K, dW.p, K, dC2.p, M, 1.0, 1.0, dS.p, nslab, &ex);
               if ( r < 0 ) rc = -r;
            }
         }
         (void) hipEventRecord(e1, 0);
         float t = 0.f;
         if ( rc == HS_OK && (hipEventSynchronize(e1) != hipSuccess || hipEventElapsedTime(&t, e0, e1) != hipSuccess) )
            rc = HS_ERR_HIP;
         *(which == 0 ? ms_tile : ms_gram) = (double) t / reps;
      }
      (void) hipEventDestroy(e0); (void) hipEventDestroy(e1);
   }
   if ( rc == HS_OK && hipDeviceSynchronize() != hipSuccess )
      rc = HS_ERR_HIP;
   (void) hipFree(dn);
   return rc;
}

extern "C" int hipsdp_gram_plan_info(int device, int M, long long K, int nslab, int* no, int* nd, int* nitems, double* span)
{
   HS_CALL( pick_device(device) );
   return hs_gram_plan_info(M, K, nslab, no, nd, nitems, span) ? HIPSDP_OK : HIPSDP_ERR_ARG;
}

extern "C" int hipsdp_schur_identity_unit(int device, int m1, int n, const double* A, double ws_gbytes, int full_storage, double* Mx,
   double* flops)
{
   HS_CALL( pick_device(device) );
   if ( m1 <= 0 || n <= 0 || A == NULL || Mx == NULL )
      return HIPSDP_ERR_ARG;
   const long long n2 = (long long) n * n;
   const long long Lp = (((long long) n * (n + 1) / 2) + 1) & ~1LL;
   DevBuf dA, dP, dM;
   HS_CALL( dA.alloc(m1 * n2) ); HS_CALL( dM.alloc((long long) m1 * m1) );
   HS_CALL( dA.up(A, m1 * n2) ); HS_CALL( dM.up(Mx, (long long) m1 * m1) );
   if ( !full_storage )
      HS_CALL( dP.alloc(m1 * Lp) );
   hs_schur_ws w;
   int rc = hs_schur_ws_alloc(&w, m1, n2, ws_gbytes > 0.0 ? ws_gbytes : 40.0);
   if ( rc != HS_OK )
   {
      hs_schur_ws_free(&w);
      return rc;
   }
   const double before = hs_mfma_flops_total();
   if ( full_storage )
      rc = hs_schur_W_identity(0, m1, n, dA.p, dM.p, &w);
   else
   {
      rc = hs_pack_rows(0, m1, n, Lp, dA.p, dP.p);
      if ( rc == HS_OK ) rc = hs_schur_W_identity_packed(0, m1, n, dP.p, Lp, dM.p, &w);
   }
   if ( flops != NULL )
      *flops = hs_mfma_flops_total() - before;
   if ( rc == HS_OK && hipDeviceSynchronize() != hipSuccess ) rc = HS_ERR_HIP;
   hs_schur_ws_free(&w);
   HS_CALL( rc );
   HS_CALL( dM.down(Mx, (long long) m1 * m1) );
   return HIPSDP_OK;
}

extern "C" int hipsdp_schur_dense(int device, int m1, int n, const double* A, const double* X, const double* Zinv, double* Mx,
   double ws_gbytes)
{
   HS_CALL( pick_device(device) );
   const long long n2 = (long long) n * n;
   DevBuf dA, dX, dZ, dM;
   HS_CALL( dA.alloc(m1 * n2) ); HS_CALL( dX.alloc(n2) ); HS_CALL( dZ.alloc(n2) ); HS_CALL( dM.alloc((long long) m1 * m1) );
   HS_CALL( dA.up(A, m1 * n2) ); HS_CALL( dX.up(X, n2) ); HS_CALL( dZ.up(Zinv, n2) );
   hs_schur_ws w;
   HS_CALL( hs_schur_ws_alloc(&w, m1, n2, ws_gbytes > 0.0 ? ws_gbytes : 1e9) );
   if ( ws_gbytes > 0.0 && w.chunk_cols > 1 )
   {
      long long cols = (long long) (ws_gbytes * 1e9 / (16.0 * (double) n2));
      if ( cols < 1 ) cols = 1;
      if ( cols < w.chunk_cols ) w.chunk_cols = cols;
   }
   HS_CALL( hs_fill(0, dM.p, (long long) m1 * m1, 0.0) );
   int rc = hs_schur_U(0, m1, n, dA.p, dX.p, dZ.p, dM.p, &w, 0, m1);
   if ( rc == HS_OK ) rc = hs_mirror_lower(0, dM.p, m1, m1);
   if ( rc == HS_OK && hipDeviceSynchronize() != hipSuccess ) rc = HS_ERR_HIP;
   hs_schur_ws_free(&w);
   HS_CALL( rc );
   HS_CALL( dM.down(Mx, (long long) m1 * m1) );
   return HIPSDP_OK;
}

extern "C" int hipsdp_schur_shard_time(int device, int m1, int n, int nranks, int rank, int by_columns, int reps, double ws_gbytes,
   double* ms)
{
   HS_CALL( pick_device(device) );
   if ( m1 < 1 || n < 1 || nranks < 1 || rank < 0 || rank >= nranks || reps < 1 || ms == NULL )
      return HIPSDP_ERR_ARG;
   const long long n2 = (long long) n * n;
   DevBuf dA, dX, dZ, dM;
   HS_CALL( dA.alloc(m1 * n2) ); HS_CALL( dX.alloc(n2) ); HS_CALL( dZ.alloc(n2) ); HS_CALL( dM.alloc((long long) (m1 + 32) * m1) );
   hipLaunchKernelGGL(k_unit_fill, dim3(1024), dim3(256), 0, 0, m1 * n2, 11ULL, dA.p);
   hipLaunchKernelGGL(k_unit_fill, dim3(1024), dim3(256), 0, 0, n2, 23ULL, dX.p);
   hipLaunchKernelGGL(k_unit_fill, dim3(1024), dim3(256), 0, 0, n2, 37ULL, dZ.p);
   hs_schur_ws w;
   int c, b1, b2, c0 = 0, cw = 0;
   hs_shard_rows(m1, nranks, rank, &c, &b1, &b2);
   hs_shard_cols(m1, n, nranks, rank, &c0, &cw);
   HS_CALL( hs_schur_ws_alloc(&w, m1, by_columns ? (long long) n * (cw > 0 ? cw : 1) : n2, ws_gbytes > 0.0 ? ws_gbytes : 40.0) );
   hipEvent_t e0, e1;
   HS_HIP( hipEventCreate(&e0) ); HS_HIP( hipEventCreate(&e1) );
   int rc = HS_OK;
   for (int it = 0; it <= reps && rc == HS_OK; ++it)
   {
      if ( it == 1 )
         rc = hipEventRecord(e0, 0) == hipSuccess ? HS_OK : HS_ERR_HIP;
      if ( rc == HS_OK ) rc = hs_fill(0, dM.p, (long long) m1 * m1, 0.0);
      if ( by_columns )
      {
         if ( rc == HS_OK ) rc = hs_schur_Wcols(0, m1, n, dA.p, dX.p, dZ.p, dM.p, &w, c0, cw);
         if ( rc == HS_OK ) rc = hs_mirror_lower(0, dM.p, m1, m1);
      }
      else
      {
         if ( rc == HS_OK ) rc = hs_schur_Urows(0, m1, n, dA.p, dX.p, dZ.p, dM.p, &w, b1, b1 + c);
         if ( rc == HS_OK ) rc = hs_schur_Urows(0, m1, n, dA.p, dX.p, dZ.p, dM.p, &w, b2, b2 + c);
         if ( rc == HS_OK ) rc = hs_mirror_upper(0, dM.p, m1, m1);
      }
   }
   float t = 0.f;
   if ( rc == HS_OK && (hipEventRecord(e1, 0) != hipSuccess || hipEventSynchronize(e1) != hipSuccess
         || hipEventElapsedTime(&t, e0, e1) != hipSuccess) )
      rc = HS_ERR_HIP;
   (void) hipEventDestroy(e0); (void) hipEventDestroy(e1);
   hs_schur_ws_free(&w);
   HS_CALL( rc );
   *ms = (double) t / (double) reps;
   return HIPSDP_OK;
}

extern "C" int hipsdp_comm_create_null(int rank, int nranks, void** comm);
extern "C" void hipsdp_comm_destroy(void* comm);
extern "C" int hipsdp_schur_var_share_time(int device, int m1, int n, int nranks, int rank, int cw, int reps, double* ms, double* a2a_bytes)
{
   HS_CALL( pick_device(device) );
   if ( m1 < 1 || n < 1 || nranks < 1 || nranks > 64 || rank < 0 || rank >= nranks || reps < 1 || ms == NULL || cw < 1 )
      return HIPSDP_ERR_ARG;
   if ( cw > n ) cw = n;
   const long long n2 = (long long) n * n;
   int r0, r1, q0, q1;
   hs_var_rows(m1, nranks, rank, &r0, &r1);
   hs_var_wrows(n, nranks, rank, &q0, &q1);
   DevBuf dA, dX, dZ, dM;
   HS_CALL( dA.alloc((long long) (r1 - r0 > 0 ? r1 - r0 : 1) * n2) ); HS_CALL( dX.alloc(n2) ); HS_CALL( dZ.alloc(n2) );
   HS_CALL( dM.alloc((long long) (m1 + 32) * m1) );
   hipLaunchKernelGGL(k_unit_fill, dim3(1024), dim3(256), 0, 0, (long long) (r1 - r0) * n2, 11ULL, dA.p);
   hipLaunchKernelGGL(k_unit_fill, dim3(1024), dim3(256), 0, 0, n2, 23ULL, dX.p);
   hipLaunchKernelGGL(k_unit_fill, dim3(1024), dim3(256), 0, 0, n2, 37ULL, dZ.p);
   void* comm = NULL;
   HS_CALL( hipsdp_comm_create_null(rank, nranks, &comm) );
   hs_schur_ws w;
   int rc = hs_schur_ws_alloc_var(&w, m1, nranks, n, cw);
   hipEvent_t e0, e1;
   HS_HIP( hipEventCreate(&e0) ); HS_HIP( hipEventCreate(&e1) );
   for (int it = 0; it <= reps && rc == HS_OK; ++it)
   {
      if ( it == 1 )
         rc = hipEventRecord(e0, 0) == hipSuccess ? HS_OK : HS_ERR_HIP;
      if ( rc == HS_OK ) rc = hs_fill(0, dM.p, (long long) m1 * m1, 0.0);
      for (int c0 = 0; c0 < n && rc == HS_OK; c0 += cw)
         rc = hs_schur_Wvar(0, comm, rank, nranks, m1, n, dA.p - (long long) r0 * n2, dX.p, dZ.p, dM.p, &w, c0, n - c0 < cw ? n - c0 : cw);
      if ( rc == HS_OK ) rc = hs_mirror_lower(0, dM.p, m1, m1);
   }
   float t = 0.f;
   if ( rc == HS_OK && (hipEventRecord(e1, 0) != hipSuccess || hipEventSynchronize(e1) != hipSuccess
         || hipEventElapsedTime(&t, e0, e1) != hipSuccess) )
      rc = HS_ERR_HIP;
   (void) hipEventDestroy(e0); (void) hipEventDestroy(e1);
   hs_schur_ws_free(&w);
   hipsdp_comm_destroy(comm);
   HS_CALL( rc );
   *ms = (double) t / (double) reps;
   if ( a2a_bytes != NULL )
      *a2a_bytes = 8.0 * (double) (r1 - r0) * (double) (n - (q1 - q0)) * (double) n;
   return HIPSDP_OK;
}

extern "C" int hipsdp_schur_w(int device, int m1, int n, const double* A, const double* X, const double* Z, double* Mx)
{
   HS_CALL( pick_device(device) );
   const long long n2 = (long long) n * n;
   DevBuf dA, dX, dZ, dG, dT, dM, dD;
   int* dflag = NULL;
   HS_CALL( dA.alloc(m1 * n2) ); HS_CALL( dX.alloc(n2) ); HS_CALL( dZ.alloc(n2) ); HS_CALL( dG.alloc(n2) ); HS_CALL( dT.alloc(n2) );
   HS_CALL( dM.alloc((long long) m1 * m1) ); HS_CALL( dD.alloc(hs_potrf_dinv_len(n)) );
   HS_HIP( hipMalloc((void**) &dflag, sizeof(int)) );
   HS_HIP( hipMemset(dflag, 0, sizeof(int)) );
   HS_CALL( dA.up(A, m1 * n2) ); HS_CALL( dX.up(X, n2) ); HS_CALL( dZ.up(Z, n2) );
   hs_schur_ws w;
   int rc = hs_schur_ws_alloc(&w, m1, n2, 1e9);
   if ( rc == HS_OK ) rc = hs_potrf(0, n, dZ.p, dD.p, dflag, NULL);
   if ( rc == HS_OK ) rc = hs_trtri(0, n, dZ.p, dD.p, dG.p, dT.p);
   if ( rc == HS_OK ) rc = hs_potrf(0, n, dX.p, dD.p, dflag, NULL);
   if ( rc == HS_OK ) rc = hs_zero_upper(0, dX.p, n);
   if ( rc == HS_OK ) rc = hs_fill(0, dM.p, (long long) m1 * m1, 0.0);
   if ( rc == HS_OK ) rc = hs_schur_W(0, m1, n, dA.p, dX.p, dG.p, dM.p, &w);
   if ( rc == HS_OK ) rc = hs_mirror_lower(0, dM.p, m1, m1);
   if ( rc == HS_OK && hipDeviceSynchronize() != hipSuccess ) rc = HS_ERR_HIP;
   hs_schur_ws_free(&w);
   (void) hipFree(dflag);
   HS_CALL( rc );
   HS_CALL( dM.down(Mx, (long long) m1 * m1) );
   return HIPSDP_OK;
}

extern "C" int hipsdp_schur_form_unit(int device, int form, int parts, int m1, int n, const double* A, const double* P, const double* Q,
   double ws_gbytes, double* Mx, int* used)
{
   HS_CALL( pick_device(device) );
   if ( form < 0 || form > 4 || m1 < 1 || n < 1 || A == NULL || P == NULL || Q == NULL || Mx == NULL || !(ws_gbytes == ws_gbytes) )
      return HIPSDP_ERR_ARG;
   if ( ((form == 1 || form == 2) && (parts < 1 || parts > 64)) || (form == 4 && parts < 1) )
      return HIPSDP_ERR_ARG;
   const long long n2 = (long long) n * n;
   if ( n2 > 2000000000LL || (long long) m1 * n > 2000000000LL || (long long) m1 * m1 > 2000000000LL )
      return HIPSDP_ERR_ARG;
   DevBuf dA, dP, dQ, dM;
   HS_CALL( dA.alloc(m1 * n2) ); HS_CALL( dP.alloc(n2) ); HS_CALL( dQ.alloc(n2) ); HS_CALL( dM.alloc((long long) m1 * m1) );
   HS_CALL( dA.up(A, m1 * n2) ); HS_CALL( dP.up(P, n2) ); HS_CALL( dQ.up(Q, n2) );
   hs_schur_ws w;
   void* comm = NULL;
   int rc = HS_OK;
   if ( form == 1 )
   {
      long long widest = 1;
      for (int g = 0; g < parts; ++g)
      {
         int c0, cw;
         hs_shard_cols(m1, n, parts, g, &c0, &cw);
         if ( (long long) n * cw > widest ) widest = (long long) n * cw;
      }
      rc = hs_schur_ws_alloc(&w, m1, widest, 40.0);
   }
   else if ( form == 4 )
   {
      if ( parts > n ) parts = n;
      rc = hipsdp_comm_create_null(0, 1, &comm);
      if ( rc != HS_OK )
         return rc;
      rc = hs_schur_ws_alloc_var(&w, m1, 1, n, parts);
   }
   else
   {
      rc = hs_schur_ws_alloc(&w, m1, n2, form == 3 && ws_gbytes > 0.0 ? ws_gbytes : 40.0);
      if ( rc == HS_OK && form == 3 && ws_gbytes > 0.0 && w.chunk_cols > 1 )
      {
         long long cols = (long long) (ws_gbytes * 1e9 / (16.0 * (double) n2));
         if ( cols < 1 ) cols = 1;
         if ( cols < w.chunk_cols ) w.chunk_cols = cols;
      }
   }
   const int t2 = hs_dgemm2_enable(1), t5 = hs_dgemm2_paired_taken(), tg = hs_gram_taken();
   if ( rc == HS_OK ) rc = hs_fill(0, dM.p, (long long) m1 * m1, 0.0);
   switch ( form )
   {
   case 0:
      if ( rc == HS_OK ) rc = hs_schur_W(0, m1, n, dA.p, dP.p, dQ.p, dM.p, &w);
      break;
   case 1:
      for (int g = 0; g < parts && rc == HS_OK; ++g)
      {
         int c0, cw;
         hs_shard_cols(m1, n, parts, g, &c0, &cw);
         rc = hs_schur_Wcols(0, m1, n, dA.p, dP.p, dQ.p, dM.p, &w, c0, cw);
      }
      break;
   case 2:
      for (int g = 0; g < parts && rc == HS_OK; ++g)
      {
         int c, b1, b2;
         hs_shard_rows(m1, parts, g, &c, &b1, &b2);
         rc = hs_schur_Urows(0, m1, n, dA.p, dP.p, dQ.p, dM.p, &w, b1, b1 + c);
         if ( rc == HS_OK ) rc = hs_schur_Urows(0, m1, n, dA.p, dP.p, dQ.p, dM.p, &w, b2, b2 + c);
      }
      break;
   case 3:
      if ( rc == HS_OK ) rc = hs_schur_U(0, m1, n, dA.p, dP.p, dQ.p, dM.p, &w, 0, m1);
      break;
   default:
      if ( rc == HS_OK ) rc = hs_schur_Wvar_all(0, NULL, comm, 0, 1, m1, n, dA.p, dP.p, dQ.p, dM.p, &w, parts, 0);
      break;
   }
   if ( rc == HS_OK ) rc = form == 2 ? hs_mirror_upper(0, dM.p, m1, m1) : hs_mirror_lower(0, dM.p, m1, m1);
   if ( rc == HS_OK && hipDeviceSynchronize() != hipSuccess ) rc = HS_ERR_HIP;
   if ( used != NULL )
   {
      used[0] = hs_dgemm2_enable(1) - t2;
      used[1] = hs_dgemm2_paired_taken() - t5;
      used[2] = hs_gram_taken() - tg;
   }
   hs_schur_ws_free(&w);
   if ( comm != NULL )
      hipsdp_comm_destroy(comm);
   HS_CALL( rc );
   HS_CALL( dM.down(Mx, (long long) m1 * m1) );
   return HIPSDP_OK;
}

extern "C" int hipsdp_schur_small_unit(int device, int m1, int nblk, const int* ns, const double* const* A, const double* const* X,
   const double* const* Zinv, int q, const double* Dext, const double* x, const double* z, double* Mx, double* Lm, double* diagM, int* taken)
{
   HS_CALL( pick_device(device) );
   if ( m1 < 1 || m1 > 32768 || nblk < 1 || nblk > 64 || ns == NULL || A == NULL || X == NULL || Zinv == NULL || q < 0 || Mx == NULL
      || Lm == NULL || diagM == NULL || taken == NULL || (q > 0 && (Dext == NULL || x == NULL || z == NULL)) )
      return HIPSDP_ERR_ARG;
   for (int k = 0; k < nblk; ++k)
      if ( ns[k] < 1 || ns[k] > 4096 || A[k] == NULL || X[k] == NULL || Zinv[k] == NULL )
         return HIPSDP_ERR_ARG;
   const int m = m1 - 1;
   std::vector<DevBuf> dA(nblk), dX(nblk), dZ(nblk);
   std::vector<const double*> pA(nblk), pX(nblk), pZ(nblk);
   for (int k = 0; k < nblk; ++k)
   {
      const long long n2 = (long long) ns[k] * ns[k];
      HS_CALL( dA[k].alloc(m1 * n2) ); HS_CALL( dX[k].alloc(n2) ); HS_CALL( dZ[k].alloc(n2) );
      HS_CALL( dA[k].up(A[k], m1 * n2) ); HS_CALL( dX[k].up(X[k], n2) ); HS_CALL( dZ[k].up(Zinv[k], n2) );
      pA[k] = dA[k].p; pX[k] = dX[k].p; pZ[k] = dZ[k].p;
   }
   DevBuf dD, dx, dz, dM, dL, dg;
   HS_CALL( dD.alloc((long long) q * m1) ); HS_CALL( dx.alloc(q) ); HS_CALL( dz.alloc(q) );
// ... 1597 lines not shown
```

Measured before the change: 13.42.

## Add wide 256-column gram kernel instance chosen by plan span

Templates the gram (W·Wᵀ) MFMA kernel into a narrow 128-tile and a wide 256x128 variant launched with 512 threads and one block per CU. The diagonal path is restructured to pick per-wave fragments at compile time. A planner builds both schedules and picks the wide one when its estimated span beats the narrow one by a gain factor and the tile count is even. The intent is more operand reuse per LDS load and fewer work items, at the cost of higher register pressure and lower occupancy. Also adds unit-test entry points and a force switch for choosing the instance.

Measured after the change: 13.69 (median of 6 runs). +2.0%, better.

```diff
diff --git a/include/hipsdp_units.h b/include/hipsdp_units.h
--- a/include/hipsdp_units.h
+++ b/include/hipsdp_units.h
@@ -21,6 +21,10 @@
 HIPSDP_API int  hipsdp_tri_product_unit(int device, int mode, int M, int N, int K, int layB, int batch, int flags, const double* A,
    const double* B, double* Cio, int crows, int ldc, int* used);
 HIPSDP_API int  hipsdp_tri_instance_force(int mode);
+HIPSDP_API int  hipsdp_gram_product_unit(int device, int mode, int M, long long K, const double* W, long long ldw, double alpha, double beta,
+   double* Cio, int nslab, int* used);
+HIPSDP_API int  hipsdp_gram_instance_force(int mode);
+HIPSDP_API int  hipsdp_gram_plan_unit(int inst, int forced, int M, long long K, int nslab, int cap, int* items, int* off, int* info);
 HIPSDP_API int  hipsdp_schur_identity_unit(int device, int m1, int n, const double* A, double ws_gbytes, int full_storage, double* Mx,
    double* flops);
 HIPSDP_API int  hipsdp_schur_dense(int device, int m1, int n, const double* A, const double* X, const double* Zinv, double* Mx,
diff --git a/scip-sdp_amd/binding.py b/scip-sdp_amd/binding.py
--- a/scip-sdp_amd/binding.py
+++ b/scip-sdp_amd/binding.py
@@ -1026,6 +1026,31 @@
     return ulib().hipsdp_tri_instance_force(mode)
 
 
+def gram_product_unit(W, K, mode, alpha=1.0, beta=0.0, Cin=None, nslab=64, device=0):
+    W = _f64(W)
+    M, ldw = W.shape
+    Cio = np.zeros((M, M)) if Cin is None else _f64(Cin).copy()
+    assert Cio.shape == (M, M)
+    used = (C.c_int * 2)(0, 0)
+    _chk(ulib().hipsdp_gram_product_unit(device, mode, M, C.c_longlong(K), _dp(W), C.c_longlong(ldw), C.c_double(alpha), C.c_double(beta),
+                                         _dp(Cio), nslab, used), "hipsdp_gram_product_unit")
+    return Cio, tuple(used)
+
+
+def gram_instance_force(mode):
+    return ulib().hipsdp_gram_instance_force(mode)
+
+
+def gram_plan_unit(inst, M, K, nslab=64, forced=False):
+    info = (C.c_int * 4)()
+    off = np.zeros(513, dtype=np.int32)
+    items = np.zeros((4096, 6), dtype=np.int32)
+    if ulib().hipsdp_gram_plan_unit(inst, int(forced), M, C.c_longlong(K), nslab, items.shape[0], _ip(items), _ip(off), info) != 0:
+        return None
+    assert info[0] <= items.shape[0]
+    return items[:info[0], :5].copy(), off[:info[1] + 1].copy(), info[2], info[3]
+
+
 def gram_selfcheck(M, K, reps=0, device=0):
     used = C.c_int(0)
     nr = C.c_longlong(0)
diff --git a/scip-sdp_amd/csrc/gram.hip b/scip-sdp_amd/csrc/gram.hip
--- a/scip-sdp_amd/csrc/gram.hip
+++ b/scip-sdp_amd/csrc/gram.hip
@@ -1,9 +1,11 @@
 #include "hs_common.h"
 #include <stdlib.h>
 #include <stdio.h>
+#include <string.h>
 #include <map>
 #include <mutex>
 #include <utility>
+#include <type_traits>
 #include <tuple>
 #include <vector>
 #include <queue>
@@ -14,12 +16,11 @@
 typedef __attribute__((address_space(3))) void* gr_lds_ptr;
 typedef const __attribute__((address_space(1))) void* gr_gbl_ptr;
 
-#define GR_BT   128
 #define GR_BKS  8
 #define GR_NS   4
-#define GR_OPSZ (GR_BT * GR_BKS)
-#define GR_SLOT (2 * GR_OPSZ)
 #define GR_GPS  4
+#define GR_BT(inst)  ((inst) ? 256 : 128)
+#define GR_NWG(inst) ((inst) ? 256 : 512)
 #define GR_UNI(x) __builtin_amdgcn_readfirstlane(x)
 
 __device__ __attribute__((aligned(16))) double hs_gr_zero[2] = {0.0, 0.0};
@@ -29,7 +30,7 @@
    int ti, tj;
    int k0, k1;
    int slab;
-   int pad;
+   int half;
 };
 
 struct gram_args
@@ -53,25 +54,33 @@
    return img[t * 128 + (k >> 1) * 32 + (lane & 15) * 2 + (k & 1)];
 }
 
-__global__ void __launch_bounds__(256, 2) hs_gram_kernel(gram_args g)
-{
+template<int WIDE>
+__global__ void __launch_bounds__(WIDE ? 512 : 256, WIDE ? 1 : 2) hs_gram_kernel(gram_args g)
+{
+   constexpr int BT = GR_BT(WIDE);
+   constexpr int OPA = BT * GR_BKS, OPB = 128 * GR_BKS, SLOT = OPA + OPB;
+   constexpr int GPS = WIDE ? 3 : GR_GPS;
+   constexpr int NSL = BT / 16;
+   constexpr int NA = 4, NB = 4, NACC = NA * NB;
+   constexpr int ND = NSL + 1;
+   constexpr int NREG = ND > NACC ? ND : NACC;
    extern __shared__ __attribute__((aligned(1024))) double gr_smem[];
    const int tid = threadIdx.x, lane = tid & 63;
    const int wave = GR_UNI(tid >> 6);
    const int wm = wave >> 1, wn = wave & 1;
-   const int wg = (blockIdx.x & 7) * 64 + (blockIdx.x >> 3);
+   const int wg = (blockIdx.x & 7) * (GR_NWG(WIDE) / 8) + (blockIdx.x >> 3);
    const int lbeg = GR_UNI(g.off[wg]), lend = GR_UNI(g.off[wg + 1]);
    const int ar = lane & 15, ac = lane >> 4;
 
-   gr_v4d acc[16];
-#pragma unroll
-   for (int i = 0; i < 16; ++i)
+   gr_v4d acc[NREG];
+#pragma unroll
+   for (int i = 0; i < NREG; ++i)
       acc[i] = (gr_v4d){0.0, 0.0, 0.0, 0.0};
 
-   int dcol[9];
-   bool dlo[9];
-#pragma unroll
-   for (int k = 0; k < 9; ++k)
+   int dcol[ND];
+   bool dlo[ND];
+#pragma unroll
+   for (int k = 0; k < ND; ++k)
    {
       dlo[k] = k <= wave;
       dcol[k] = k <= wave ? k : k - wave - 1;
@@ -83,86 +92,83 @@
    auto piece = [&](int st, int k) __attribute__((always_inline))
    {
       const int i = k & 1;
-      const int pc = wave * 2 + i;
+      const int pc = (WIDE && k >= 2) ? wave : wave * 2 + i;
       const int K0 = ck0 + GR_BKS * st;
       const double* src = (K0 + 2 * ac < ck1) ? (k < 2 ? pa[i] : pb[i]) + K0 : hs_gr_zero;
-      __builtin_amdgcn_global_load_lds((gr_gbl_ptr) src, (gr_lds_ptr) (gr_smem + (st & 3) * GR_SLOT + (k < 2 ? 0 : GR_OPSZ) + pc * 128), 16, 0, 0);
+      __builtin_amdgcn_global_load_lds((gr_gbl_ptr) src, (gr_lds_ptr) (gr_smem + (st & 3) * SLOT + (k < 2 ? 0 : OPA) + pc * 128), 16, 0, 0);
    };
 
    auto run_off = [&](int nst) __attribute__((always_inline))
    {
-      double f0a[4], f0b[4], f1a[4], f1b[4];
-      auto landed_frags = [&](double (&fa)[4], double (&fb)[4]) __attribute__((always_inline))
-      {
-#pragma unroll
-         for (int i = 0; i < 4; ++i)
-            asm volatile("" : "+v"(fa[i]), "+v"(fb[i]));
+      double f0a[NA], f0b[NB], f1a[NA], f1b[NB];
+      auto landed_frags = [&](double (&fa)[NA], double (&fb)[NB]) __attribute__((always_inline))
+      {
+#pragma unroll
+         for (int i = 0; i < NA; ++i)
+            asm volatile("" : "+v"(fa[i]));
+#pragma unroll
+         for (int i = 0; i < NB; ++i)
+            asm volatile("" : "+v"(fb[i]));
       };
+      auto read_frags = [&](double (&fa)[NA], double (&fb)[NB], const double* img, int ks) __attribute__((always_inline))
+      {
+#pragma unroll
+         for (int i = 0; i < NA; ++i)
+            fa[i] = gr_frag(img, NA * wm + i, ks, lane);
+#pragma unroll
+         for (int i = 0; i < NB; ++i)
+            fb[i] = gr_frag(img + OPA, NB * wn + i, ks, lane);
+      };
 #pragma unroll
       for (int st = 0; st < GR_NS; ++st)
 #pragma unroll
-         for (int k = 0; k < 4; ++k)
+         for (int k = 0; k < GPS; ++k)
             piece(st, k);
-      gr_wait_vm<3 * 4>();
+      gr_wait_vm<3 * GPS>();
       __builtin_amdgcn_s_barrier();
-#pragma unroll
-      for (int i = 0; i < 4; ++i)
-      {
-         f0a[i] = gr_frag(gr_smem, 4 * wm + i, 0, lane);
-         f0b[i] = gr_frag(gr_smem + GR_OPSZ, 4 * wn + i, 0, lane);
-      }
+      read_frags(f0a, f0b, gr_smem, 0);
       asm volatile("s_waitcnt lgkmcnt(0)" ::: "memory");
       landed_frags(f0a, f0b);
       for (int s = 0; s < nst; ++s)
       {
-         const double* sa = gr_smem + (s & 3) * GR_SLOT;
-         const double* sn = gr_smem + ((s + 1) & 3) * GR_SLOT;
-         __builtin_amdgcn_sched_barrier(0);
-#pragma unroll
-         for (int i = 0; i < 4; ++i)
-         {
-            f1a[i] = gr_frag(sa, 4 * wm + i, 1, lane);
-            f1b[i] = gr_frag(sa + GR_OPSZ, 4 * wn + i, 1, lane);
-         }
-#pragma unroll
-         for (int i = 0; i < 4; ++i)
-#pragma unroll
-            for (int j = 0; j < 4; ++j)
-               acc[4 * i + j] = __builtin_amdgcn_mfma_f64_16x16x4f64(f0a[i], f0b[j], acc[4 * i + j], 0, 0, 0);
-#pragma unroll
-         for (int q = 0; q < 8; ++q)
+         const double* sa = gr_smem + (s & 3) * SLOT;
+         const double* sn = gr_smem + ((s + 1) & 3) * SLOT;
+         __builtin_amdgcn_sched_barrier(0);
+         read_frags(f1a, f1b, sa, 1);
+#pragma unroll
+         for (int i = 0; i < NA; ++i)
+#pragma unroll
+            for (int j = 0; j < NB; ++j)
+               acc[NB * i + j] = __builtin_amdgcn_mfma_f64_16x16x4f64(f0a[i], f0b[j], acc[NB * i + j], 0, 0, 0);
+#pragma unroll
+         for (int q = 0; q < NA + NB; ++q)
          {
             __builtin_amdgcn_sched_group_barrier(0x008, 1, 0);
             __builtin_amdgcn_sched_group_barrier(0x100, 1, 0);
          }
-         __builtin_amdgcn_sched_group_barrier(0x008, 8, 0);
+         __builtin_amdgcn_sched_group_barrier(0x008, NACC - NA - NB, 0);
          __builtin_amdgcn_sched_barrier(0);
          asm volatile("s_waitcnt lgkmcnt(0)" ::: "memory");
          landed_frags(f1a, f1b);
-         gr_wait_vm<2 * 4>();
+         gr_wait_vm<2 * GPS>();
          __builtin_amdgcn_s_barrier();
          __builtin_amdgcn_sched_barrier(0);
          acc[0] = __builtin_amdgcn_mfma_f64_16x16x4f64(f1a[0], f1b[0], acc[0], 0, 0, 0);
          acc[1] = __builtin_amdgcn_mfma_f64_16x16x4f64(f1a[0], f1b[1], acc[1], 0, 0, 0);
 #pragma unroll
-         for (int k = 0; k < 4; ++k)
+         for (int k = 0; k < GPS; ++k)
          {
             __builtin_amdgcn_sched_barrier(0);
             piece(s + GR_NS, k);
-            acc[2 + k] = __builtin_amdgcn_mfma_f64_16x16x4f64(f1a[(2 + k) >> 2], f1b[(2 + k) & 3], acc[2 + k], 0, 0, 0);
-         }
-         __builtin_amdgcn_sched_barrier(0);
-#pragma unroll
-         for (int i = 0; i < 4; ++i)
-         {
-            f0a[i] = gr_frag(sn, 4 * wm + i, 0, lane);
-            f0b[i] = gr_frag(sn + GR_OPSZ, 4 * wn + i, 0, lane);
-         }
-#pragma unroll
-         for (int k = 6; k < 16; ++k)
-            acc[k] = __builtin_amdgcn_mfma_f64_16x16x4f64(f1a[k >> 2], f1b[k & 3], acc[k], 0, 0, 0);
-#pragma unroll
-         for (int q = 0; q < 8; ++q)
+            acc[2 + k] = __builtin_amdgcn_mfma_f64_16x16x4f64(f1a[(2 + k) / NB], f1b[(2 + k) % NB], acc[2 + k], 0, 0, 0);
+         }
+         __builtin_amdgcn_sched_barrier(0);
+         read_frags(f0a, f0b, sn, 0);
+#pragma unroll
+         for (int k = 2 + GPS; k < NACC; ++k)
+            acc[k] = __builtin_amdgcn_mfma_f64_16x16x4f64(f1a[k / NB], f1b[k % NB], acc[k], 0, 0, 0);
+#pragma unroll
+         for (int q = 0; q < NA + NB; ++q)
          {
             __builtin_amdgcn_sched_group_barrier(0x008, 1, 0);
             __builtin_amdgcn_sched_group_barrier(0x100, 1, 0);
@@ -173,28 +179,26 @@
       }
    };
 
-   auto run_diag = [&](int nst) __attribute__((always_inline))
-   {
-      double a0[2], b0[9], a1[2], b1[9];
-      auto read_set = [&](double (&a)[2], double (&b)[9], const double* img, int ks) __attribute__((always_inline))
-      {
-         a[0] = gr_frag(img, wave, ks, lane);
-         a[1] = gr_frag(img, 7 - wave, ks, lane);
-#pragma unroll
-         for (int k = 0; k < 9; ++k)
-            b[k] = gr_frag(img, dcol[k], ks, lane);
+   auto run_diag = [&](auto wsel, int nst) __attribute__((always_inline))
+   {
+      constexpr int W0 = decltype(wsel)::value, W1 = NSL - 1 - W0;
+      constexpr int CM = (W0 > W1 ? W0 : W1) + 1;
+      double f0[CM], f1[CM];
+      auto read_set = [&](double (&f)[CM], const double* img, int ks, int c0, int c1) __attribute__((always_inline))
+      {
+#pragma unroll
+         for (int c = c0; c < c1; ++c)
+            f[c] = gr_frag(img, c, ks, lane);
       };
-      auto landed_set = [&](double (&a)[2], double (&b)[9]) __attribute__((always_inline))
-      {
-         asm volatile("" : "+v"(a[0]), "+v"(a[1]));
-#pragma unroll
-         for (int k = 0; k < 9; ++k)
-            asm volatile("" : "+v"(b[k]));
+      auto landed_set = [&](double (&f)[CM]) __attribute__((always_inline))
+      {
+#pragma unroll
+         for (int c = 0; c < CM; ++c)
+            asm volatile("" : "+v"(f[c]));
       };
-      auto mfma_k = [&](const double (&a)[2], const double (&b)[9], int k) __attribute__((always_inline))
-      {
-         const double av = dlo[k] ? a[0] : a[1];
-         acc[k] = __builtin_amdgcn_mfma_f64_16x16x4f64(av, b[k], acc[k], 0, 0, 0);
+      auto mfma_k = [&](const double (&f)[CM], int k) __attribute__((always_inline))
+      {
+         acc[k] = __builtin_amdgcn_mfma_f64_16x16x4f64(f[k <= W0 ? W0 : W1], f[k <= W0 ? k : k - W0 - 1], acc[k], 0, 0, 0);
       };
 #pragma unroll
       for (int st = 0; st < GR_NS; ++st)
@@ -203,57 +207,61 @@
             piece(st, k);
       gr_wait_vm<3 * 2>();
       __builtin_amdgcn_s_barrier();
-      read_set(a0, b0, gr_smem, 0);
+      read_set(f0, gr_smem, 0, 0, CM);
       asm volatile("s_waitcnt lgkmcnt(0)" ::: "memory");
-      landed_set(a0, b0);
+      landed_set(f0);
       for (int s = 0; s < nst; ++s)
       {
-         const double* sa = gr_smem + (s & 3) * GR_SLOT;
-         const double* sn = gr_smem + ((s + 1) & 3) * GR_SLOT;
-         __builtin_amdgcn_sched_barrier(0);
-         read_set(a1, b1, sa, 1);
-#pragma unroll
-         for (int k = 0; k < 9; ++k)
-            mfma_k(a0, b0, k);
-#pragma unroll
-         for (int q = 0; q < 5; ++q)
+         const double* sa = gr_smem + (s & 3) * SLOT;
+         const double* sn = gr_smem + ((s + 1) & 3) * SLOT;
+         __builtin_amdgcn_sched_barrier(0);
+         read_set(f1, sa, 1, 0, CM);
+#pragma unroll
+         for (int k = 0; k < ND; ++k)
+            mfma_k(f0, k);
+#pragma unroll
+         for (int q = 0; q < CM; ++q)
+         {
+            __builtin_amdgcn_sched_group_barrier(0x008, 1, 0);
+            __builtin_amdgcn_sched_group_barrier(0x100, 1, 0);
+         }
+         __builtin_amdgcn_sched_group_barrier(0x008, ND - CM, 0);
+         __builtin_amdgcn_sched_barrier(0);
+         asm volatile("s_waitcnt lgkmcnt(0)" ::: "memory");
+         landed_set(f1);
+         gr_wait_vm<2 * 2>();
+         __builtin_amdgcn_s_barrier();
+         __builtin_amdgcn_sched_barrier(0);
+         read_set(f0, sn, 0, 0, 4);
+         mfma_k(f1, 0);
+         mfma_k(f1, 1);
+#pragma unroll
+         for (int q = 0; q < 2; ++q)
          {
             __builtin_amdgcn_sched_group_barrier(0x008, 1, 0);
             __builtin_amdgcn_sched_group_barrier(0x100, 2, 0);
          }
-         __builtin_amdgcn_sched_group_barrier(0x008, 1, 0);
-         __builtin_amdgcn_sched_group_barrier(0x100, 1, 0);
-         __builtin_amdgcn_sched_group_barrier(0x008, 3, 0);
-         __builtin_amdgcn_sched_barrier(0);
-         asm volatile("s_waitcnt lgkmcnt(0)" ::: "memory");
-         landed_set(a1, b1);
-         gr_wait_vm<2 * 2>();
-         __builtin_amdgcn_s_barrier();
-         __builtin_amdgcn_sched_barrier(0);
-         mfma_k(a1, b1, 0);
-         mfma_k(a1, b1, 1);
 #pragma unroll
          for (int k = 0; k < 2; ++k)
          {
             __builtin_amdgcn_sched_barrier(0);
             piece(s + GR_NS, k);
-            mfma_k(a1, b1, 2 + k);
-         }
-         __builtin_amdgcn_sched_barrier(0);
-         read_set(a0, b0, sn, 0);
-#pragma unroll
-         for (int k = 4; k < 9; ++k)
-            mfma_k(a1, b1, k);
-#pragma unroll
-         for (int q = 0; q < 4; ++q)
+            mfma_k(f1, 2 + k);
+         }
+         __builtin_amdgcn_sched_barrier(0);
+         read_set(f0, sn, 0, 4, CM);
+#pragma unroll
+         for (int k = 4; k < ND; ++k)
+            mfma_k(f1, k);
+#pragma unroll
+         for (int q = 0; q < (CM - 4 + 1) / 2; ++q)
          {
             __builtin_amdgcn_sched_group_barrier(0x008, 1, 0);
-            __builtin_amdgcn_sched_group_barrier(0x100, 3, 0);
-         }
-         __builtin_amdgcn_sched_group_barrier(0x008, 1, 0);
+            __builtin_amdgcn_sched_group_barrier(0x100, 2, 0);
+         }
          __builtin_amdgcn_sched_barrier(0);
          asm volatile("s_waitcnt lgkmcnt(0)" ::: "memory");
-         landed_set(a0, b0);
+         landed_set(f0);
       }
    };
 
@@ -264,48 +272,63 @@
       ck0 = GR_UNI(it.k0); ck1 = GR_UNI(it.k1);
       const int nst = (ck1 - ck0 + GR_BKS - 1) / GR_BKS;
       const bool diag = cti == ctj;
+      const int n0 = ctj * BT + (WIDE ? 128 * GR_UNI(it.half) : 0);
 #pragma unroll
       for (int i = 0; i < 2; ++i)
       {
          const int pc = wave * 2 + i;
-         int row = cti * GR_BT + pc * 16 + ar;
+         int row = cti * BT + pc * 16 + ar;
          if ( row > g.M - 1 ) row = g.M - 1;
          pa[i] = g.W + (long long) row * g.ldw + 2 * ac;
-         int rowb = ctj * GR_BT + pc * 16 + ar;
+         int rowb = n0 + (WIDE ? wave : pc) * 16 + ar;
          if ( rowb > g.M - 1 ) rowb = g.M - 1;
          pb[i] = g.W + (long long) rowb * g.ldw + 2 * ac;
       }
       if ( diag )
-         run_diag(nst);
+      {
+#define GR_DIAG_CASE(w) case w: run_diag(std::integral_constant<int, w>(), nst); break
+         if constexpr ( WIDE )
+            switch ( wave )
+            {
+               GR_DIAG_CASE(0); GR_DIAG_CASE(1); GR_DIAG_CASE(2); GR_DIAG_CASE(3);
+               GR_DIAG_CASE(4); GR_DIAG_CASE(5); GR_DIAG_CASE(6); default: run_diag(std::integral_constant<int, 7>(), nst); break;
+            }
+         else
+            switch ( wave )
+            {
+               GR_DIAG_CASE(0); GR_DIAG_CASE(1); GR_DIAG_CASE(2); default: run_diag(std::integral_constant<int, 3>(), nst); break;
+            }
+#undef GR_DIAG_CASE
+      }
       else
          run_off(nst);
       gr_wait_vm<0>();
       {
          double* C = g.ws + (long long) cslab * (long long) g.M * g.M;
-         const int m0 = cti * GR_BT, n0 = ctj * GR_BT;
+         const int m0 = cti * BT;
          if ( !diag )
          {
 #pragma unroll
-            for (int i = 0; i < 4; ++i)
+            for (int i = 0; i < NA; ++i)
 #pragma unroll
                for (int r = 0; r < 4; ++r)
                {
-                  const int row = m0 + wm * 64 + 16 * i + (lane >> 4) + 4 * r;
+                  const int row = m0 + wm * (16 * NA) + 16 * i + (lane >> 4) + 4 * r;
                   if ( row < g.M )
                   {
                      double* cr = C + (long long) row * g.M + n0 + wn * 64 + (lane & 15);
 #pragma unroll
-                     for (int j = 0; j < 4; ++j)
-                        cr[16 * j] = acc[4 * i + j][r];
+                     for (int j = 0; j < NB; ++j)
+                        cr[16 * j] = acc[NB * i + j][r];
                   }
                }
          }
          else
          {
 #pragma unroll
-            for (int k = 0; k < 9; ++k)
+            for (int k = 0; k < ND; ++k)
             {
-               const int rs = dlo[k] ? wave : 7 - wave;
+               const int rs = dlo[k] ? wave : NSL - 1 - wave;
 #pragma unroll
                for (int r = 0; r < 4; ++r)
                {
@@ -317,14 +340,14 @@
             }
          }
 #pragma unroll
-         for (int i = 0; i < 16; ++i)
+         for (int i = 0; i < NREG; ++i)
             acc[i] = (gr_v4d){0.0, 0.0, 0.0, 0.0};
       }
       __syncthreads();
    }
 }
 
-__global__ void hs_gram_reduce_kernel(int M, int no, int nd, const double* __restrict__ ws, double* __restrict__ C, long long ldc, double alpha, double beta)
+__global__ void hs_gram_reduce_kernel(int M, int bt, int no, int nd, const double* __restrict__ ws, double* __restrict__ C, long long ldc, double alpha, double beta)
 {
    const long long MM = (long long) M * M;
    for (long long e = (long long) blockIdx.x * blockDim.x + threadIdx.x; e < MM; e += (long long) gridDim.x * blockDim.x)
@@ -332,7 +355,7 @@
       const int r = (int) (e / M), c = (int) (e - (long long) r * M);
       if ( c > r )
          continue;
-      const int ns = (r / GR_BT == c / GR_BT) ? nd : no;
+      const int ns = (r / bt == c / bt) ? nd : no;
       double s = 0.0;
       for (int k = 0; k < ns; ++k)
          s += ws[(long long) k * MM + e];
@@ -347,6 +370,7 @@
 {
    std::vector<gram_item> items;
    std::vector<int> off;
+   int inst;
    int no, nd;
    double span;
    double executed;
@@ -354,45 +378,55 @@
    int* devoff;
 };
 
-#define GR_DIAG_COST 0.72
-
-bool gr_make_plan(GramPlan& P, int tm, long long K, int so, int sd)
-{
-   const int noff = tm * (tm - 1) / 2;
-   const double cd = GR_DIAG_COST;
+#ifndef GR_DIAG_COST_WIDE
+#define GR_DIAG_COST_WIDE 1.06
+#endif
+#ifndef GR_DIAG_COST_128
+#define GR_DIAG_COST_128 0.72
+#endif
+#define GR_DIAG_COST(inst) ((inst) ? GR_DIAG_COST_WIDE : GR_DIAG_COST_128)
+#ifndef GR_WIDE_GAIN
+#define GR_WIDE_GAIN 0.96
+#endif
+
+bool gr_make_plan(GramPlan& P, int inst, int tm, long long K, int so, int sd)
+{
+   const double cd = GR_DIAG_COST(inst);
+   const int nwg = GR_NWG(inst), wpx = nwg / 8;
    if ( so < 1 || sd < 1 )
       return false;
    long long lo = (K + so - 1) / so, ld = (K + sd - 1) / sd;
    lo = ((lo + GR_BKS - 1) / GR_BKS) * GR_BKS;
    ld = ((ld + GR_BKS - 1) / GR_BKS) * GR_BKS;
-   if ( (long long) (so - 1) * lo + 8 * GR_BKS > K || (long long) (sd - 1) * ld + 8 * GR_BKS > K )
+   if ( (so > 1 && (long long) (so - 1) * lo + 8 * GR_BKS > K) || (sd > 1 && (long long) (sd - 1) * ld + 8 * GR_BKS > K) )
       return false;
    std::vector<gram_item> all;
    for (int s = 0; s < so; ++s)
       for (int i = 1; i < tm; ++i)
          for (int j = 0; j < i; ++j)
-         {
-            gram_item it = {i, j, (int) (s * lo), (int) ((s + 1) * lo < K ? (s + 1) * lo : K), s, 0};
-            all.push_back(it);
-         }
+            for (int h = 0; h <= inst; ++h)
+            {
+               gram_item it = {i, j, (int) (s * lo), (int) ((s + 1) * lo < K ? (s + 1) * lo : K), s, h};
+               all.push_back(it);
+            }
    for (int s = 0; s < sd; ++s)
       for (int i = 0; i < tm; ++i)
       {
          gram_item it = {i, i, (int) (s * ld), (int) ((s + 1) * ld < K ? (s + 1) * ld : K), s, 0};
          all.push_back(it);
       }
-   (void) noff;
    std::stable_sort(all.begin(), all.end(), [](const gram_item& a, const gram_item& b) { return a.k0 < b.k0; });
    auto cost = [&](const gram_item& it) { return (it.ti == it.tj ? cd : 1.0) * (double) (it.k1 - it.k0) / (double) K; };
+   const double mo = inst ? 256.0 : 128.0, md = inst ? 272.0 : 72.0;
    double total = 0.0;
    P.executed = 0.0;
    for (const gram_item& it : all)
    {
       total += cost(it);
-      P.executed += 2048.0 * (double) ((it.k1 - it.k0 + GR_BKS - 1) / GR_BKS) * (it.ti == it.tj ? 72.0 : 128.0);
+      P.executed += 2048.0 * (double) ((it.k1 - it.k0 + GR_BKS - 1) / GR_BKS) * (it.ti == it.tj ? md : mo);
    }
    P.items.clear();
-   P.off.assign(513, 0);
+   P.off.assign(nwg + 1, 0);
    P.span = 0.0;
    size_t pos = 0;
    double done = 0.0;
@@ -408,43 +442,35 @@
       std::vector<size_t> order(mine.size());
       for (size_t i = 0; i < order.size(); ++i) order[i] = i;
       std::stable_sort(order.begin(), order.end(), [&](size_t a, size_t b) { return cost(mine[a]) > cost(mine[b]); });
-      std::vector<std::vector<gram_item> > lists(64);
-      std::vector<double> load(64, 0.0);
+      std::vector<std::vector<gram_item> > lists(wpx);
+      std::vector<double> load(wpx, 0.0);
       for (size_t i : order)
       {
          int w = 0;
-         for (int v = 1; v < 64; ++v)
+         for (int v = 1; v < wpx; ++v)
             if ( load[v] < load[w] ) w = v;
          load[w] += cost(mine[i]);
          lists[w].push_back(mine[i]);
       }
-      for (int w = 0; w < 64; ++w)
+      for (int w = 0; w < wpx; ++w)
       {
          std::stable_sort(lists[w].begin(), lists[w].end(), [](const gram_item& a, const gram_item& b) { return a.k0 < b.k0; });
-         P.off[64 * x + w] = (int) P.items.size();
+         P.off[wpx * x + w] = (int) P.items.size();
          for (const gram_item& it : lists[w])
             P.items.push_back(it);
          if ( load[w] > P.span ) P.span = load[w];
       }
    }
-   P.off[512] = (int) P.items.size();
+   P.off[nwg] = (int) P.items.size();
+   P.inst = inst;
    P.no = so; P.nd = sd;
    return true;
 }
 
-GramPlan* gr_plan(int M, long long K, int nslab)
-{
-   static std::mutex mu;
-   static std::map<std::tuple<int, int, long long, int>, GramPlan*> tab;
-   int dev = 0;
-   if ( hipGetDevice(&dev) != hipSuccess )
-      return NULL;
-   std::lock_guard<std::mutex> lk(mu);
-   const auto key = std::make_tuple(dev, M, K, nslab);
-   auto f = tab.find(key);
-   if ( f != tab.end() )
-      return f->second;
-   const int tm = (M + GR_BT - 1) / GR_BT;
+GramPlan* gr_build(int M, long long K, int nslab, int inst, bool forced)
+{
+   const int bt = GR_BT(inst), nwg = GR_NWG(inst);
+   const int tm = (M + bt - 1) / bt;
    const int ntile = tm * (tm + 1) / 2;
    GramPlan* best = NULL;
    GramPlan cand;
@@ -461,28 +487,51 @@
          *best = cand;
       }
    };
-   const int noff = ntile - tm;
-   for (int so = 1; so <= nslab && (long long) noff * so + tm <= 512; ++so)
-      for (int sd = (so + 1) / 2; sd <= so && (long long) noff * so + (long long) tm * sd <= 512; ++sd)
-         consider(gr_make_plan(cand, tm, K, so, sd), 0.24 * ((double) so * noff + (double) sd * tm) / (double) K);
+   const int noff = (ntile - tm) * (inst ? 2 : 1);
+   for (int so = 1; so <= nslab && (long long) noff * so + tm <= nwg; ++so)
+      for (int sd = inst ? so : (so + 1) / 2; sd <= (inst ? 2 * so : so) && sd <= nslab && (long long) noff * so + (long long) tm * sd <= nwg; ++sd)
+         consider(gr_make_plan(cand, inst, tm, K, so, sd), 0.24 * ((double) so * noff + (double) sd * tm) / (double) K);
+   if ( forced )
+   {
+      if ( best == NULL )
+         consider(gr_make_plan(cand, inst, tm, K, 1, 1), 0.0);
+      return best;
+   }
    if ( best != NULL )
    {
-      const int sold = hs_dgemm_pick_xcd_slices(ntile, K);
-      const double oldspan = (double) (((long long) ntile * sold + 511) / 512) / (double) sold;
-      if ( best->span * 1.03 > oldspan || best->items.size() < 256 )
+      const int t128 = (M + 127) / 128, n128 = t128 * (t128 + 1) / 2;
+      const int sold = hs_dgemm_pick_xcd_slices(n128, K);
+      const double oldspan = (double) (((long long) n128 * sold + 511) / 512) / (double) sold;
+      if ( (inst ? GR_WIDE_GAIN : 1.0) * best->span * 1.03 > oldspan || (int) best->items.size() < nwg / 2 )
       {
          delete best;
          best = NULL;
       }
    }
+   return best;
+}
+
+GramPlan* gr_plan(int M, long long K, int nslab, int inst, bool forced)
+{
+   static std::mutex mu;
+   static std::map<std::tuple<int, int, long long, int, int>, GramPlan*> tab;
+   int dev = 0;
+   if ( hipGetDevice(&dev) != hipSuccess )
+      return NULL;
+   std::lock_guard<std::mutex> lk(mu);
+   const auto key = std::make_tuple(dev, M, K, nslab, 2 * inst + (forced ? 1 : 0));
+   auto f = tab.find(key);
+   if ( f != tab.end() )
+      return f->second;
+   GramPlan* best = gr_build(M, K, nslab, inst, forced);
    if ( best != NULL )
    {
       gram_item* d = NULL;
       int* doff = NULL;
       if ( hipMalloc((void**) &d, best->items.size() * sizeof(gram_item)) != hipSuccess
          || hipMemcpy(d, best->items.data(), best->items.size() * sizeof(gram_item), hipMemcpyHostToDevice) != hipSuccess
-         || hipMalloc((void**) &doff, 513 * sizeof(int)) != hipSuccess
-         || hipMemcpy(doff, best->off.data(), 513 * sizeof(int), hipMemcpyHostToDevice) != hipSuccess )
+         || hipMalloc((void**) &doff, best->off.size() * sizeof(int)) != hipSuccess
+         || hipMemcpy(doff, best->off.data(), best->off.size() * sizeof(int), hipMemcpyHostToDevice) != hipSuccess )
       {
          if ( d != NULL ) (void) hipFree(d);
          if ( doff != NULL ) (void) hipFree(doff);
@@ -496,53 +545,105 @@
    return best;
 }
 
-}
-
-static int gr_taken = 0;
+int gr_inst_mode = -1;
+int gr_taken = 0;
+int gr_wide_taken = 0;
+
+GramPlan* gr_choose(int M, long long K, int nslab)
+{
+   const int mode = gr_inst_mode;
+   if ( mode >= 0 )
+      return gr_plan(M, K, nslab, mode, true);
+   GramPlan* P = gr_plan(M, K, nslab, 0, false);
+   if ( P == NULL || P->dev == NULL || (((M + 127) / 128) & 1) )
+      return P;
+   GramPlan* Pw = gr_plan(M, K, nslab, 1, false);
+   if ( Pw != NULL && Pw->dev != NULL && GR_WIDE_GAIN * Pw->span <= P->span )
+      return Pw;
+   return P;
+}
+
+}
 
 int hs_gram_taken(void)
 {
    return __atomic_load_n(&gr_taken, __ATOMIC_RELAXED);
+}
+
+int hs_gram_instance_force(int mode)
+{
+   if ( mode >= -1 && mode <= 1 )
+      gr_inst_mode = mode;
+   return __atomic_load_n(&gr_wide_taken, __ATOMIC_RELAXED);
 }
 
 int hs_gram_try(hipStream_t stream, int M, long long K, const double* W, long long ldw, double* C, long long ldc, double alpha, double beta,
    double* ws, int nslab, double* executed)
 {
-   if ( ws == NULL || nslab < 2 || M < 256 || K < 16384 )
+   const bool forced = gr_inst_mode >= 0;
+   if ( ws == NULL || nslab < 2 || M < 1 || K < 2 || (!forced && (M < 256 || K < 16384)) )
       return 0;
    if ( (ldw & 1) || (K & 1) || (((uintptr_t) W) & 15) || K > 2000000000LL )
       return 0;
    if ( nslab > 64 ) nslab = 64;
-   GramPlan* P = gr_plan(M, K, nslab);
-   if ( P == NULL || P->dev == NULL || P->items.size() < 256 )
+   GramPlan* P = gr_choose(M, K, nslab);
+   if ( P == NULL || P->dev == NULL || P->items.empty() )
       return 0;
    gram_args g;
    g.W = W; g.ldw = ldw; g.M = M; g.ws = ws; g.items = P->dev; g.off = P->devoff;
-   static hs_attr_mask attr_done;
-   const size_t smem = (size_t) GR_NS * GR_SLOT * sizeof(double);
-   if ( hs_func_max_lds(reinterpret_cast<const void*>(&hs_gram_kernel), (int) smem, &attr_done) != HS_OK )
-      return -HS_ERR_HIP;
-   hipLaunchKernelGGL(hs_gram_kernel, dim3(512), dim3(256), smem, stream, g);
+   const size_t smem = (size_t) GR_NS * (GR_BT(P->inst) + 128) * GR_BKS * sizeof(double);
+   if ( P->inst )
+   {
+      static hs_attr_mask attr_wide;
+      if ( hs_func_max_lds(reinterpret_cast<const void*>(&hs_gram_kernel<1>), (int) smem, &attr_wide) != HS_OK )
+         return -HS_ERR_HIP;
+      hipLaunchKernelGGL(hs_gram_kernel<1>, dim3(GR_NWG(1)), dim3(512), smem, stream, g);
+   }
+   else
+   {
+      static hs_attr_mask attr_done;
+      if ( hs_func_max_lds(reinterpret_cast<const void*>(&hs_gram_kernel<0>), (int) smem, &attr_done) != HS_OK )
+         return -HS_ERR_HIP;
+      hipLaunchKernelGGL(hs_gram_kernel<0>, dim3(GR_NWG(0)), dim3(256), smem, stream, g);
+   }
    if ( hipGetLastError() != hipSuccess )
       return -HS_ERR_HIP;
    {
       int blocks = (int) (((long long) M * M + 255) / 256);
       if ( blocks > 2048 ) blocks = 2048;
-      hipLaunchKernelGGL(hs_gram_reduce_kernel, dim3(blocks), dim3(256), 0, stream, M, P->no, P->nd, ws, C, ldc, alpha, beta);
+      hipLaunchKernelGGL(hs_gram_reduce_kernel, dim3(blocks), dim3(256), 0, stream, M, GR_BT(P->inst), P->no, P->nd, ws, C, ldc, alpha, beta);
       if ( hipGetLastError() != hipSuccess )
          return -HS_ERR_HIP;
    }
    if ( executed != NULL )
       *executed = P->executed;
    (void) __atomic_add_fetch(&gr_taken, 1, __ATOMIC_RELAXED);
+   if ( P->inst )
+      (void) __atomic_add_fetch(&gr_wide_taken, 1, __ATOMIC_RELAXED);
    return 1;
 }
 
 int hs_gram_plan_info(int M, long long K, int nslab, int* no, int* nd, int* nitems, double* span)
 {
-   GramPlan* P = gr_plan(M, K, nslab > 64 ? 64 : nslab);
+   GramPlan* P = gr_choose(M, K, nslab > 64 ? 64 : nslab);
    if ( P == NULL )
       return 0;
    *no = P->no; *nd = P->nd; *nitems = (int) P->items.size(); *span = P->span;
    return 1;
 }
+
+int hs_gram_plan_host(int inst, int forced, int M, long long K, int nslab, int cap, int* items, int* off, int* info)
+{
+   if ( inst < 0 || inst > 1 || M < 1 || K < 2 || nslab < 1 )
+      return 0;
+   GramPlan* P = gr_build(M, K, nslab > 64 ? 64 : nslab, inst, forced != 0);
+   if ( P == NULL )
+      return 0;
+   info[0] = (int) P->items.size(); info[1] = GR_NWG(inst); info[2] = P->no; info[3] = P->nd;
+   for (size_t i = 0; i < P->off.size(); ++i)
+      off[i] = P->off[i];
+   for (int i = 0; i < info[0] && i < cap; ++i)
+      memcpy(items + 6 * (size_t) i, &P->items[i], sizeof(gram_item));
+   delete P;
+   return 1;
+}
diff --git a/scip-sdp_amd/csrc/hs_common.h b/scip-sdp_amd/csrc/hs_common.h
--- a/scip-sdp_amd/csrc/hs_common.h
+++ b/scip-sdp_amd/csrc/hs_common.h
@@ -90,10 +90,12 @@
 int hs_dgemm2_wide_force(int mode);
 int hs_dgemm2_tri5_forced(void);
 int hs_gram_taken(void);
+int hs_gram_instance_force(int mode);
 
 int hs_gram_try(hipStream_t stream, int M, long long K, const double* W, long long ldw, double* C, long long ldc, double alpha, double beta,
    double* ws, int nslab, double* executed);
 int hs_gram_plan_info(int M, long long K, int nslab, int* no, int* nd, int* nitems, double* span);
+int hs_gram_plan_host(int inst, int forced, int M, long long K, int nslab, int cap, int* items, int* off, int* info);
 
 int hs_dgemm3_try(hipStream_t stream, const hs_gemm_args* args);
 
diff --git a/scip-sdp_amd/csrc/units.hip b/scip-sdp_amd/csrc/units.hip
--- a/scip-sdp_amd/csrc/units.hip
+++ b/scip-sdp_amd/csrc/units.hip
@@ -367,6 +367,41 @@
 {
    HS_CALL( pick_device(device) );
    return hs_gram_plan_info(M, K, nslab, no, nd, nitems, span) ? HIPSDP_OK : HIPSDP_ERR_ARG;
+}
+
+extern "C" int hipsdp_gram_product_unit(int device, int mode, int M, long long K, const double* W, long long ldw, double alpha, double beta,
+   double* Cio, int nslab, int* used)
+{
+   HS_CALL( pick_device(device) );
+   if ( mode < -1 || mode > 1 || M < 1 || K < 1 || ldw < K || W == NULL || Cio == NULL || nslab < 1 || nslab > 64 || used == NULL )
+      return HIPSDP_ERR_ARG;
+   const long long MM = (long long) M * M;
+   DevBuf dW, dC, dS;
+   HS_CALL( dW.alloc((long long) M * ldw) ); HS_CALL( dC.alloc(MM) ); HS_CALL( dS.alloc((long long) nslab * MM) );
+   HS_CALL( dW.up(W, (long long) M * ldw) ); HS_CALL( dC.up(Cio, MM) );
+   hipLaunchKernelGGL(k_unit_fill, dim3(1024), dim3(256), 0, 0, (long long) nslab * MM, 52ULL, dS.p);
+   const int tg = hs_gram_taken();
+   const int tw = hs_gram_instance_force(mode);
+   const int r = hs_gram_try(0, M, K, dW.p, ldw, dC.p, M, alpha, beta, dS.p, nslab, NULL);
+   int rc = r < 0 ? -r : HS_OK;
+   if ( rc == HS_OK && hipDeviceSynchronize() != hipSuccess ) rc = HS_ERR_HIP;
+   used[1] = hs_gram_instance_force(-1) - tw;
+   used[0] = hs_gram_taken() - tg;
+   HS_CALL( rc );
+   HS_CALL( dC.down(Cio, MM) );
+   return HIPSDP_OK;
+}
+
+extern "C" int hipsdp_gram_instance_force(int mode)
+{
+   return hs_gram_instance_force(mode);
+}
+
+extern "C" int hipsdp_gram_plan_unit(int inst, int forced, int M, long long K, int nslab, int cap, int* items, int* off, int* info)
+{
+   if ( items == NULL || off == NULL || info == NULL || cap < 0 )
+      return HIPSDP_ERR_ARG;
+   return hs_gram_plan_host(inst, forced, M, K, nslab, cap, items, off, info) ? HIPSDP_OK : HIPSDP_ERR_ARG;
 }
 
 extern "C" int hipsdp_schur_identity_unit(int device, int m1, int n, const double* A, double ws_gbytes, int full_storage, double* Mx,
```
